# ForJadeForest/DistillCLIP

Hardware: AMD Instinct MI355X
Metric: image-text pairs/sec (distill step) (higher is better)
Workload: dtype bf16; 1 GPU; l_clip.yaml dual distill: ViT-B/32 CLIP teacher -> weight-shared ViT(6x768,24h,R2) + text(4x768,12h,R2) students, 224px/77tok, losses out_l1+out_cos+0.1*cos_diff, fwd+loss+bwd+AdamW; global_batch=512, batch_per_gpu=512, parallelism=dp1, gradient_exchange=none, negatives=local (reference training_step semantics), optimizer_in_step=True, teacher_residual=fp16, saved_gelu_derivative=u8 fixed point, clock_probe=True

## Files before the change

### distillclip_amd/csrc/attention_mix.hip

```cpp
#include <math.h>
#include <stdlib.h>
#include "common.h"

#define DEVFN __device__ __forceinline__
#define DEVMEM __device__ __forceinline__
typedef __attribute__((ext_vector_type(8))) _Float16 f16x8;

namespace hw {
DEVFN f32x4 mfma_bf16(bf16x8 a, bf16x8 b, f32x4 c) { return __builtin_amdgcn_mfma_f32_16x16x32_bf16(a, b, c, 0, 0, 0); }
DEVFN f32x4 mfma_f16(f16x8 a, f16x8 b, f32x4 c) { return __builtin_amdgcn_mfma_f32_16x16x32_f16(a, b, c, 0, 0, 0); }
DEVFN float exp2(float x) { return __builtin_amdgcn_exp2f(x); }
DEVFN float log2(float x) { return __builtin_amdgcn_logf(x); }
DEVFN bool any(bool p) { return __builtin_amdgcn_ballot_w64(p) != 0; }
DEVFN void lds_fence() { wave_lds_fence(); }
DEVFN void block_sync() { __syncthreads(); }
template <int OFF>
DEVFN bf16x8 lds_read_frag(const char* p) {
    bf16x8 v;
    asm volatile("ds_read_b128 %0, %1 offset:%2" : "=v"(v) : "v"((unsigned)(uintptr_t)p), "n"(OFF));
    return v;
}
template <int N, int GF>
DEVFN void lds_wait_frags(bf16x8 (&f)[GF]) {
    static_assert(GF == 4 || GF == 8, "fragment group of 4 or 8");
    if constexpr (GF == 8)
        asm volatile("s_waitcnt lgkmcnt(%8)" : "+v"(f[0]), "+v"(f[1]), "+v"(f[2]), "+v"(f[3]), "+v"(f[4]), "+v"(f[5]), "+v"(f[6]), "+v"(f[7]) : "n"(N));
    else
        asm volatile("s_waitcnt lgkmcnt(%4)" : "+v"(f[0]), "+v"(f[1]), "+v"(f[2]), "+v"(f[3]) : "n"(N));
}
DEVFN void pin_acc(bf16x8& v) { asm volatile("" : "+a"(v)); }
DEVFN unsigned long long clock() { return __builtin_readcyclecounter(); }
template <class T8> DEVFN void keep_alive(const T8 (&f)[4]) { mfma_keep_alive(f); }
template <class T8> DEVFN void keep_alive(const T8& f) { mfma_keep_alive(f); }
DEVFN void mfma_src_guard() { __builtin_amdgcn_sched_barrier(0); asm volatile("s_nop 7\n\ts_nop 3" ::: "memory"); __builtin_amdgcn_sched_barrier(0); }
DEVFN void sched_fence() { __builtin_amdgcn_sched_barrier(0); }
typedef __attribute__((address_space(3))) void lds_void;
typedef __attribute__((address_space(1))) const void gbl_void;
DEVFN void dma16(const void* src, char* dst) { __builtin_amdgcn_global_load_lds((gbl_void*)src, (lds_void*)dst, 16, 0, 0); }
template <int N> DEVFN void dma_wait() { asm volatile("s_waitcnt vmcnt(%0)" ::"n"(N) : "memory"); }
}

#include "attn_mix_wave.h"

namespace {

constexpr int BWD_MAX_WG = 256;

DEVFN int pick_tile(const int32_t* pick, int b, int N) {
    const int it = (pick[b] - b * N) >> 4;
    return __builtin_amdgcn_readfirstlane(min(max(it, 0), (N - 1) >> 4));
}

template <int H, int HD, int OCC, bool PICK = false>
__global__ __launch_bounds__(256, OCC) void attn_mix_fwd_kernel(amix::FwdArgs p, const int32_t* pick) {
    using C = amix::Cfg<H, HD>;
    extern __shared__ __attribute__((aligned(16))) char smem[];
    const int lane = threadIdx.x & 63;
    const int wave = __builtin_amdgcn_readfirstlane(threadIdx.x >> 6);
    const int item = blockIdx.x * 4 + wave;
    if (item >= (PICK ? p.B : p.B * p.QT)) return;
    const int b = PICK ? item : item / p.QT, it = PICK ? pick_tile(pick, b, p.N) : item - b * p.QT;
    const unsigned long long te = p.stamps ? hw::clock() : 0;
    char* lds = smem + wave * amix::fwd_lds_per_wave<C>();
    amix::zero_block_init<C>(lds, lane);
    amix::FwdWeights<C> w;
    amix::fwd_load_weights<C>(p, lane, w);
    if (p.stamps && lane == 0) {
        p.stamps[12 * (long)item + 8] = hw::clock() - te;
        p.stamps[12 * (long)item + 10] = __builtin_amdgcn_s_memrealtime();
    }
    amix::fwd_item<C>(p, b, it, lane, w, lds);
    if (p.stamps && lane == 0) p.stamps[12 * (long)item + 11] = __builtin_amdgcn_s_memrealtime();
}

template <class C, bool PASS_B>
DEVFN void bwd_wave_pick(const amix::BwdArgs& p, const int32_t* pick, int wg, int nwg, int wave, int nwave, int lane, char* lds_all) {
    using namespace amix;
    constexpr int RT = C::RT, HP = C::HP;
    constexpr int PER_WAVE = bwd_lds_per_wave<C>(), TILE_OFF = bwd_tile_off<C>();
    char* lds = lds_all + wave * PER_WAVE;
    for (int o = lane * 16; o < 2 * WG_TILE; o += 64 * 16) *(u32x4*)(lds + TILE_OFF + o) = u32x4{0u, 0u, 0u, 0u};
    zero_block_init<C>(lds, lane);
    BwdWeights<C> w;
    bwd_load_weights<C, PASS_B>(p, lane, w);
    f32x4 acc[RT][RT];
#pragma unroll
    for (int t = 0; t < RT; ++t)
#pragma unroll
        for (int u = 0; u < RT; ++u) acc[t][u] = f32x4{0.f, 0.f, 0.f, 0.f};
    for (int b = wg * nwave + wave; b < p.B; b += nwg * nwave) bwd_item<C, PASS_B>(p, b, pick_tile(pick, b, p.N), lane, w, acc, lds);
    hw::lds_fence();
    float* mine = (float*)(lds + TILE_OFF);
    const int c = lane & 15, g4 = lane >> 4;
#pragma unroll
    for (int t = 0; t < RT; ++t)
#pragma unroll
        for (int u = 0; u < RT; ++u)
#pragma unroll
            for (int r = 0; r < 4; ++r) mine[(16 * t + 4 * g4 + r) * HP + 16 * u + c] = acc[t][u][r];
    hw::block_sync();
    float* out = p.partial + ((long)wg * 2 + (PASS_B ? 0 : 1)) * HP * HP;
    for (int idx = wave * 64 + lane; idx < HP * HP; idx += nwave * 64) {
        float s = 0.f;
        for (int v = 0; v < nwave; ++v) s += ((const float*)(lds_all + v * PER_WAVE + TILE_OFF))[idx];
        out[idx] = s;
    }
}

template <int H, int HD, bool PASS_B, bool PICK = false>
__global__ __launch_bounds__(256) void attn_mix_bwd_kernel(amix::BwdArgs p, const int32_t* pick) {
    using C = amix::Cfg<H, HD>;
    extern __shared__ __attribute__((aligned(16))) char smem[];
    const int lane = threadIdx.x & 63;
    const int wave = __builtin_amdgcn_readfirstlane(threadIdx.x >> 6);
    if constexpr (PICK) bwd_wave_pick<C, PASS_B>(p, pick, blockIdx.x, gridDim.x, wave, 4, lane, smem);
    else amix::bwd_wave<C, PASS_B>(p, blockIdx.x, gridDim.x, wave, 4, lane, smem);
}

__global__ __launch_bounds__(256) void attn_mix_wgrad_reduce_kernel(const float* __restrict__ partial, int nwg, int H, int HP, float* dWl, float* dWw) {
    __shared__ float part[4];
    const int idx = blockIdx.x;
    const int which = idx / (H * H), gh = idx - which * H * H, g = gh / H, h = gh - g * H;
    const int w = threadIdx.x;
    float v = w < nwg ? partial[((size_t)w * 2 + which) * HP * HP + g * HP + h] : 0.f;
    v = wave_sum(v);
    if ((w & 63) == 0) part[w >> 6] = v;
    __syncthreads();
    if (w == 0) {
        float* dst = which == 0 ? dWl : dWw;
        dst[gh] += (part[0] + part[1]) + (part[2] + part[3]);
    }
}

unsigned long long* g_fwd_stamps = nullptr;
unsigned long long* g_bwd_stamps[2] = {nullptr, nullptr};

}

#define MIX_DISPATCH(Hv, HDv, ...)                                                     \
    switch ((Hv) * 100 + (HDv)) {                                                      \
        case 232: { constexpr int HH = 2, HD_ = 32; typedef amix::Cfg<HH, HD_> CC; __VA_ARGS__; break; }              \
        case 264: { constexpr int HH = 2, HD_ = 64; typedef amix::Cfg<HH, HD_> CC; __VA_ARGS__; break; }              \
        case 432: { constexpr int HH = 4, HD_ = 32; typedef amix::Cfg<HH, HD_> CC; __VA_ARGS__; break; }              \
        case 464: { constexpr int HH = 4, HD_ = 64; typedef amix::Cfg<HH, HD_> CC; __VA_ARGS__; break; }              \
        case 832: { constexpr int HH = 8, HD_ = 32; typedef amix::Cfg<HH, HD_> CC; __VA_ARGS__; break; }              \
        case 864: { constexpr int HH = 8, HD_ = 64; typedef amix::Cfg<HH, HD_> CC; __VA_ARGS__; break; }              \
        case 1232: { constexpr int HH = 12, HD_ = 32; typedef amix::Cfg<HH, HD_> CC; __VA_ARGS__; break; }            \
        case 1264: { constexpr int HH = 12, HD_ = 64; typedef amix::Cfg<HH, HD_> CC; __VA_ARGS__; break; }            \
        case 2432: { constexpr int HH = 24, HD_ = 32; typedef amix::Cfg<HH, HD_> CC; __VA_ARGS__; break; }            \
        default: dclip_set_error("attn_mix: no instantiation for H=%d hd=%d", (int)(Hv), (int)(HDv)); return DCLIP_EINVAL; \
    }

extern "C" int dclip_attn_mix_supported(int64_t H, int64_t N, int64_t hd) {
    const bool shape = ((H == 2 || H == 4 || H == 8 || H == 12) && (hd == 32 || hd == 64)) || (H == 24 && hd == 32);
    return shape && H * hd <= 1024 && (H * hd) % 128 == 0 && N >= 1 && N <= 128;
}

extern "C" void dclip_attn_mix_debug_stamps(void* fwd, void* bwd_a, void* bwd_b) {
    g_fwd_stamps = (unsigned long long*)fwd;
    g_bwd_stamps[0] = (unsigned long long*)bwd_a;
    g_bwd_stamps[1] = (unsigned long long*)bwd_b;
}

static size_t partial_bytes(int64_t H) {
    const size_t HP = (size_t)((H + 15) / 16) * 16;
    return (size_t)BWD_MAX_WG * 2 * HP * HP * sizeof(float);
}
extern "C" size_t dclip_attn_mix_bwd_workspace_bytes(int64_t B, int64_t H, int64_t N) {
    return partial_bytes(H) + (((size_t)B * H * N * sizeof(float) + 255) & ~(size_t)255);
}

namespace {

int launch_mix_fwd(const char* who, const void* qkv, int64_t ld, const float* Wl, const float* Ww, void* R, float* stats, int64_t B, int64_t H,
                   int64_t N, int64_t Np, int64_t hd, float scale, const int32_t* pick, void* stream) {
    DCLIP_REQUIRE(qkv && Wl && Ww && R && stats && B > 0, "%s: null / empty argument", who);
    DCLIP_REQUIRE(dclip_attn_mix_supported(H, N, hd), "%s: unsupported shape H=%ld N=%ld hd=%ld", who, (long)H, (long)N, (long)hd);
    DCLIP_REQUIRE(Np == ((N + 7) & ~(int64_t)7) && ld % 8 == 0 && ld >= 3 * H * hd && ((uintptr_t)qkv % 16) == 0 && ((uintptr_t)R % 16) == 0,
                  "%s: misaligned buffers (Np = round_up(N, 8), 16-byte aligned qkv rows and R)", who);
    const int QT = (int)((N + 15) / 16);
    amix::FwdArgs p{(const bf16_t*)qkv, (long)ld, Wl, Ww, (bf16_t*)R, stats, (int)B, (int)N, (int)Np, QT, scale, pick ? nullptr : g_fwd_stamps};
    const int64_t nitem = pick ? B : B * QT;
    const dim3 grid((unsigned)((nitem + 3) / 4));
    const double rows = pick ? 16.0 : (double)N, el = (double)B * H * rows * Np;
    TraceScope tr(DCLIP_TRACE_ATTN, 4.0 * B * H * rows * N * hd + 8.0 * el * H, 2.0 * el + 2.0 * B * (N + rows) * H * hd, stream, (int)(B * H), (int)N, (int)hd, 7);
    if (pick) {
        MIX_DISPATCH(H, hd, hipLaunchKernelGGL((attn_mix_fwd_kernel<HH, HD_, 2, true>), grid, dim3(256), (size_t)4 * amix::fwd_lds_per_wave<CC>(),
                                               (hipStream_t)stream, p, pick));
    } else {
        MIX_DISPATCH(H, hd, hipLaunchKernelGGL((attn_mix_fwd_kernel<HH, HD_, 2>), grid, dim3(256), (size_t)4 * amix::fwd_lds_per_wave<CC>(),
                                               (hipStream_t)stream, p, nullptr));
    }
    return dclip_check_launch(who);
}

int launch_mix_bwd(const char* who, const void* qkv, int64_t ld, const void* dO, int64_t ldo, const float* Wl, const float* Ww, const float* stats,
                   void* dS, float* dWl, float* dWw, void* workspace, size_t ws_bytes, int64_t B, int64_t H, int64_t N, int64_t Np, int64_t hd,
                   float scale, const int32_t* pick, void* stream) {
    DCLIP_REQUIRE(qkv && dO && Wl && Ww && stats && dS && dWl && dWw && workspace && B > 0, "%s: null / empty argument", who);
    DCLIP_REQUIRE(dclip_attn_mix_supported(H, N, hd), "%s: unsupported shape H=%ld N=%ld hd=%ld", who, (long)H, (long)N, (long)hd);
    DCLIP_REQUIRE(Np == ((N + 7) & ~(int64_t)7) && ld % 8 == 0 && ldo % 8 == 0 && ld >= 3 * H * hd && ldo >= H * hd && ((uintptr_t)qkv % 16) == 0 &&
                      ((uintptr_t)dO % 16) == 0 && ((uintptr_t)dS % 16) == 0 && ((uintptr_t)workspace % 16) == 0,
                  "%s: misaligned buffers", who);
    DCLIP_REQUIRE(ws_bytes >= dclip_attn_mix_bwd_workspace_bytes(B, H, N), "%s: workspace too small (%zu < %zu)", who, ws_bytes,
                  dclip_attn_mix_bwd_workspace_bytes(B, H, N));
    const int QT = (int)((N + 15) / 16);
    const int HP = (int)((H + 15) / 16) * 16;
    const int64_t nitem = pick ? B : B * QT;
    int blocks = (int)((nitem + 3) / 4);
    if (blocks > BWD_MAX_WG) blocks = BWD_MAX_WG;
    amix::BwdArgs p{(const bf16_t*)qkv, (long)ld, (const bf16_t*)dO, (long)ldo, Wl, Ww, stats, (bf16_t*)dS, (float*)workspace,
                    (float*)((char*)workspace + partial_bytes(H)), (int)B, (int)N, (int)Np, QT, scale, pick ? nullptr : g_bwd_stamps[0]};
    const double rows = pick ? 16.0 : (double)N, el = (double)B * H * rows * Np;
    TraceScope tr(DCLIP_TRACE_ATTN, 8.0 * B * H * rows * N * hd + 20.0 * el * H, 2.0 * el + 4.0 * B * (N + rows) * H * hd, stream, (int)(B * H), (int)N, (int)hd, 8);
    if (pick) {
        MIX_DISPATCH(H, hd, hipLaunchKernelGGL((attn_mix_bwd_kernel<HH, HD_, false, true>), dim3(blocks), dim3(256), (size_t)4 * amix::bwd_lds_per_wave<CC>(),
                                               (hipStream_t)stream, p, pick));
        MIX_DISPATCH(H, hd, hipLaunchKernelGGL((attn_mix_bwd_kernel<HH, HD_, true, true>), dim3(blocks), dim3(256), (size_t)4 * amix::bwd_lds_per_wave<CC>(),
                                               (hipStream_t)stream, p, pick));
    } else {
        MIX_DISPATCH(H, hd, hipLaunchKernelGGL((attn_mix_bwd_kernel<HH, HD_, false>), dim3(blocks), dim3(256), (size_t)4 * amix::bwd_lds_per_wave<CC>(),
                                               (hipStream_t)stream, p, nullptr));
        p.stamps = g_bwd_stamps[1];
        MIX_DISPATCH(H, hd, hipLaunchKernelGGL((attn_mix_bwd_kernel<HH, HD_, true>), dim3(blocks), dim3(256), (size_t)4 * amix::bwd_lds_per_wave<CC>(),
                                               (hipStream_t)stream, p, nullptr));
    }
    static_assert(BWD_MAX_WG <= 256, "one partial per thread of the reduction block");
    hipLaunchKernelGGL(attn_mix_wgrad_reduce_kernel, dim3((unsigned)(2 * H * H)), dim3(256), 0, (hipStream_t)stream,
                       (const float*)workspace, blocks, (int)H, HP, dWl, dWw);
    return dclip_check_launch(who);
}

}

extern "C" int dclip_attn_mix_fwd(const void* qkv, int64_t ld, const float* Wl, const float* Ww, void* R, float* stats, int64_t B,
                                  int64_t H, int64_t N, int64_t Np, int64_t hd, float scale, void* stream) {
    return launch_mix_fwd("dclip_attn_mix_fwd", qkv, ld, Wl, Ww, R, stats, B, H, N, Np, hd, scale, nullptr, stream);
}

extern "C" int dclip_attn_mix_bwd(const void* qkv, int64_t ld, const void* dO, int64_t ldo, const float* Wl, const float* Ww,
                                  const float* stats, void* dS, float* dWl, float* dWw, void* workspace, size_t ws_bytes, int64_t B,
                                  int64_t H, int64_t N, int64_t Np, int64_t hd, float scale, void* stream) {
    return launch_mix_bwd("dclip_attn_mix_bwd", qkv, ld, dO, ldo, Wl, Ww, stats, dS, dWl, dWw, workspace, ws_bytes, B, H, N, Np, hd, scale, nullptr, stream);
}

extern "C" int dclip_attn_mix_fwd_rows(const void* qkv, int64_t ld, const float* Wl, const float* Ww, void* R, float* stats, int64_t B,
                                       int64_t H, int64_t N, int64_t Np, int64_t hd, float scale, const int32_t* pick, void* stream) {
    DCLIP_REQUIRE(pick, "dclip_attn_mix_fwd_rows: null pick");
    return launch_mix_fwd("dclip_attn_mix_fwd_rows", qkv, ld, Wl, Ww, R, stats, B, H, N, Np, hd, scale, pick, stream);
}

extern "C" int dclip_attn_mix_bwd_rows(const void* qkv, int64_t ld, const void* dO, int64_t ldo, const float* Wl, const float* Ww,
                                       const float* stats, void* dS, float* dWl, float* dWw, void* workspace, size_t ws_bytes, int64_t B,
                                       int64_t H, int64_t N, int64_t Np, int64_t hd, float scale, const int32_t* pick, void* stream) {
    DCLIP_REQUIRE(pick, "dclip_attn_mix_bwd_rows: null pick");
    return launch_mix_bwd("dclip_attn_mix_bwd_rows", qkv, ld, dO, ldo, Wl, Ww, stats, dS, dWl, dWw, workspace, ws_bytes, B, H, N, Np, hd, scale, pick, stream);
}
```

### distillclip_amd/csrc/common.h

```cpp
#pragma once
#include <hip/hip_runtime.h>
#include <stdint.h>

typedef __bf16 bf16_t;
typedef __attribute__((ext_vector_type(8))) __bf16 bf16x8;
typedef __attribute__((ext_vector_type(4))) __bf16 bf16x4;
typedef __attribute__((ext_vector_type(2))) __bf16 bf16x2;
typedef __attribute__((ext_vector_type(8))) _Float16 f16x8;
typedef __attribute__((ext_vector_type(4))) _Float16 f16x4;
typedef __attribute__((ext_vector_type(4))) short s16x4;
typedef __attribute__((ext_vector_type(4))) float f32x4;
typedef __attribute__((ext_vector_type(16))) float f32x16;
typedef __attribute__((ext_vector_type(4))) unsigned int u32x4;

#include "dclip.h"

void dclip_set_error(const char* fmt, ...);

#define DCLIP_REQUIRE(cond, ...)                 \
    do {                                          \
        if (!(cond)) {                            \
            dclip_set_error(__VA_ARGS__);         \
            return DCLIP_EINVAL;                  \
        }                                         \
    } while (0)

extern "C" int dclip_rows_pick(const void* src, void* dst, const int32_t* idx, int64_t B, int64_t row_bytes, void* stream);
extern "C" int dclip_rows_expand(const void* src, void* dst, const int32_t* idx, int64_t B, int64_t N, int64_t row_bytes, void* stream);

extern "C" int dclip_cast_bf16_pad(const float* src, void* dst, int64_t R, int64_t C, int64_t ldd, void* stream);

bool dclip_trace_open(int kind, double flops, double bytes, void* stream, int* slot, int d0 = 0, int d1 = 0, int d2 = 0, int d3 = 0);
void dclip_trace_close(int slot, void* stream);
struct TraceScope {
    int slot = -1; void* st;
    TraceScope(int kind, double flops, double bytes, void* stream, int d0 = 0, int d1 = 0, int d2 = 0, int d3 = 0) : st(stream) {
        if (!dclip_trace_open(kind, flops, bytes, stream, &slot, d0, d1, d2, d3)) slot = -1;
    }
    ~TraceScope() { if (slot >= 0) dclip_trace_close(slot, st); }
};
#define DCLIP_TRACE_GEMM_NT 0
#define DCLIP_TRACE_GEMM_TN 1
#define DCLIP_TRACE_LAYERNORM 2
#define DCLIP_TRACE_LOSS 3
#define DCLIP_TRACE_ATTN 4
#define DCLIP_TRACE_LN_BWD 5

void dclip_explain_hip_error(const char* what, int hip_error, const char* hip_text);
static inline int dclip_check_launch(const char* what) {
    hipError_t e = hipGetLastError();
    if (e != hipSuccess) {
        dclip_explain_hip_error(what, (int)e, hipGetErrorString(e));
        return DCLIP_ELAUNCH;
    }
    return DCLIP_OK;
}

static inline int grid_for(int64_t work, int per_block = 256, int cap = 2048 * 4) {
    int64_t g = (work + per_block - 1) / per_block;
    return (int)(g < 1 ? 1 : (g > cap ? cap : g));
}

static inline size_t dclip_up256(size_t x) { return (x + 255) & ~(size_t)255; }
static inline bool dclip_aligned16(const void* p) { return ((uintptr_t)p % 16) == 0; }
struct Bump {
    char* base; size_t off;
    explicit Bump(void* b) : base((char*)b), off(0) {}
    template <class T> T* take(size_t n) {
        T* p = base ? (T*)(base + off) : nullptr;
        off += dclip_up256(n * sizeof(T));
        return p;
    }
};

__device__ __forceinline__ float bf2f(bf16_t x) { return (float)x; }
__device__ __forceinline__ bf16_t f2bf(float x) { return (bf16_t)x; }

__device__ __forceinline__ float wave_sum(float v) {
#pragma unroll
    for (int o = 32; o > 0; o >>= 1) v += __shfl_xor(v, o);
    return v;
}
__device__ __forceinline__ float wave_max(float v) {
#pragma unroll
    for (int o = 32; o > 0; o >>= 1) v = fmaxf(v, __shfl_xor(v, o));
    return v;
}

__device__ __forceinline__ void wave_lds_fence() { __builtin_amdgcn_wave_barrier(); asm volatile("" ::: "memory"); __builtin_amdgcn_wave_barrier(); }

template <class T> __device__ __forceinline__ void mfma_keep_alive(const T& f) { asm volatile("" :: "v"(f)); }
template <class T> __device__ __forceinline__ void mfma_keep_alive(const T (&f)[2]) { asm volatile("" :: "v"(f[0]), "v"(f[1])); }
template <class T> __device__ __forceinline__ void mfma_keep_alive(const T (&f)[4]) { asm volatile("" :: "v"(f[0]), "v"(f[1]), "v"(f[2]), "v"(f[3])); }

__device__ __forceinline__ float quick_gelu_f(float x) { return x * __builtin_amdgcn_rcpf(1.f + __expf(-1.702f * x)); }
__device__ __forceinline__ float erf_tail(float ax_over_sqrt2, float phi) {
    const float t = __builtin_amdgcn_rcpf(fmaf(0.3275911f, ax_over_sqrt2, 1.f));
    float p = fmaf(1.061405429f, t, -1.453152027f);
    p = fmaf(p, t, 1.421413741f);
    p = fmaf(p, t, -0.284496736f);
    p = fmaf(p, t, 0.254829592f);
    return p * t * phi;
}
__device__ __forceinline__ float gelu_erf_f(float x) {
    const float phi = __expf(-0.5f * x * x);
    const float tail = erf_tail(fabsf(x) * 0.70710678118654752f, phi);
    const float cdf = x >= 0.f ? 1.f - 0.5f * tail : 0.5f * tail;
    return x * cdf;
}
__device__ __forceinline__ float dgelu_erf_f(float x) {
    const float phi = __expf(-0.5f * x * x);
    const float tail = erf_tail(fabsf(x) * 0.70710678118654752f, phi);
    const float cdf = x >= 0.f ? 1.f - 0.5f * tail : 0.5f * tail;
    return fmaf(x * phi, 0.3989422804014327f, cdf);
}

__device__ __forceinline__ void gelu_erf_both_f(float x, float& g, float& dg) {
    const float phi = __expf(-0.5f * x * x);
    const float tail = erf_tail(fabsf(x) * 0.70710678118654752f, phi);
    const float cdf = x >= 0.f ? 1.f - 0.5f * tail : 0.5f * tail;
    g = x * cdf;
    dg = fmaf(x * phi, 0.3989422804014327f, cdf);
}

#define DCLIP_DG_LO (-0.13f)
#define DCLIP_DG_STEP (1.26f / 255.f)
__device__ __forceinline__ unsigned dg_pack4(float a, float b, float c, float d) {
    const float inv = 255.f / 1.26f, off = 0.13f * (255.f / 1.26f);
    unsigned r = 0;
    r = __builtin_amdgcn_cvt_pk_u8_f32(__builtin_rintf(fmaf(a, inv, off)), 0, r);
    r = __builtin_amdgcn_cvt_pk_u8_f32(__builtin_rintf(fmaf(b, inv, off)), 1, r);
    r = __builtin_amdgcn_cvt_pk_u8_f32(__builtin_rintf(fmaf(c, inv, off)), 2, r);
    r = __builtin_amdgcn_cvt_pk_u8_f32(__builtin_rintf(fmaf(d, inv, off)), 3, r);
    return r;
}
__device__ __forceinline__ float dg_unpack(unsigned w, int byte) {
    return fmaf((float)((w >> (8 * byte)) & 0xffu), DCLIP_DG_STEP, DCLIP_DG_LO);
}

__device__ __forceinline__ bf16x8 frag_halves(s16x4 lo, s16x4 hi) {
    union { struct { s16x4 lo, hi; } s; bf16x8 v; } u;
    u.s.lo = lo; u.s.hi = hi;
    return u.v;
}

typedef __attribute__((address_space(3))) s16x4 lds_s16x4;
template <int ROWB>
__device__ __forceinline__ bf16x8 tr_frag(const char* tile, int r0, int x0, int lane) {
    const int g = lane >> 4, q = (lane >> 2) & 3, pp = lane & 3;
    const char* a0 = tile + (r0 + 8 * g + q) * ROWB + (x0 + 4 * pp) * 2;
    return frag_halves(__builtin_amdgcn_ds_read_tr16_b64_v4i16((lds_s16x4*)a0), __builtin_amdgcn_ds_read_tr16_b64_v4i16((lds_s16x4*)(a0 + 4 * ROWB)));
}

__device__ __forceinline__ int xcd_remap(int bid, int nwg) {
    const int q = nwg >> 3, r = nwg & 7, x = bid & 7;
    return (x < r ? x * (q + 1) : r * (q + 1) + (x - r) * q) + (bid >> 3);
}
```

### distillclip_amd/csrc/encoder.cpp

```cpp
#include <math.h>
#include <stdlib.h>
#include <string.h>
#include <new>
#include <vector>
#include "common.h"

namespace {

#define CK(expr)                      \
    do {                              \
        int _rc = (expr);             \
        if (_rc != DCLIP_OK) return _rc; \
    } while (0)

enum { P_PER_TBLOCK = 12, P_PER_SBLOCK = 8, P_PER_SREPEAT = 6 };

struct Plan {
    dclip_encoder_cfg c;
    int D, H, hd, N, Np, F, E, L, R;
    int K;
    int Kp;
    bool student, image, compressed;
    bool mixing;
    bool train;
    struct EmbP { int table, w, bias, cls, pos, ln_w, ln_b; } emb;
    int p_blocks;
    struct HeadP { int norm_w, norm_b, head_w, head_b; } head;
    int n_params;
    struct BlockW { int64_t qkv, qkv_t, proj, proj_t, fc1, fc1_t, fc2, fc2_t; };
    std::vector<BlockW> bw;
    int64_t w_embed, w_embed_t, w_head, w_head_t, w_total;
};

int64_t wtake(int64_t& off, int64_t n) { int64_t o = off; off += (n + 127) & ~(int64_t)127; return o; }

bool make_plan(const dclip_encoder_cfg& c, Plan& p) {
    p.c = c;
    p.student = c.kind == 1; p.train = c.kind != 0; p.image = c.modality == 0; p.mixing = p.student && c.head_mix;
    p.D = c.width; p.H = c.heads; p.N = c.tokens; p.F = c.mlp_dim; p.E = c.out_dim; p.L = c.layers; p.R = c.repeats;
    if (c.kind < 0 || c.kind > 2 || c.modality < 0 || c.modality > 1) { dclip_set_error("encoder: bad kind/modality"); return false; }
    if (p.D <= 0 || p.H <= 0 || p.D % p.H) { dclip_set_error("encoder: width %d not divisible by heads %d", p.D, p.H); return false; }
    p.hd = p.D / p.H;
    if (p.hd != 32 && p.hd != 64) { dclip_set_error("encoder: head dim %d unsupported (32 or 64)", p.hd); return false; }
    if (p.D % 64 || p.F % 64 || p.E % 64 || p.D > 1024) { dclip_set_error("encoder: width/mlp/out dims must be multiples of 64, width <= 1024"); return false; }
    const bool long_ok = c.kind == 0 && p.image && !c.causal && p.hd == 64;
    if (p.N <= 0 || p.N > (long_ok ? 640 : 128)) {
        if (long_ok) dclip_set_error("encoder: tokens must be in 1..640 for a frozen image tower (got %d)", p.N);
        else if (p.N > 128 && c.kind != 0) dclip_set_error("encoder: tokens must be in 1..128 for a trainable tower (kind %d; got %d): only frozen image towers run longer sequences", c.kind, p.N);
        else if (p.N > 128 && !p.image) dclip_set_error("encoder: tokens must be in 1..128 for a text tower (got %d): only frozen image towers run longer sequences", p.N);
        else if (p.N > 128) dclip_set_error("encoder: tokens must be in 1..128 for a causal or head-dim-%d tower (got %d): longer sequences need a non-causal tower with head dim 64", p.hd, p.N);
        else dclip_set_error("encoder: tokens must be in 1..128 (got %d)", p.N);
        return false;
    }
    if (p.L <= 0 || p.R <= 0 || (!p.student && p.R != 1)) { dclip_set_error("encoder: bad layers/repeats"); return false; }
    p.Np = (p.N + 7) & ~7;
    p.compressed = !p.image && c.embed_rank > 0;
    p.K = p.Kp = 0;
    if (p.image) {
        if (c.patch <= 0 || c.resolution < c.patch || c.in_chans <= 0) { dclip_set_error("encoder: bad patch geometry"); return false; }
        const int g = c.resolution / c.patch;
        if (g * g + 1 != p.N) { dclip_set_error("encoder: tokens %d != (res/patch)^2 + 1 = %d", p.N, g * g + 1); return false; }
        p.K = c.in_chans * c.patch * c.patch;
        p.Kp = p.K;
        if (p.K % 64) {
            if (p.train) { dclip_set_error("encoder: in_chans*patch^2 = %d must be a multiple of 64 in a trainable tower", p.K); return false; }
            if (c.patch % 2) { dclip_set_error("encoder: patch %d must be even", c.patch); return false; }
            p.Kp = (p.K + 63) & ~63;
        }
    } else {
        if (c.vocab <= 0) { dclip_set_error("encoder: vocab required for text"); return false; }
        if (p.compressed && c.embed_rank % 64) { dclip_set_error("encoder: embed_rank must be a multiple of 64"); return false; }
        if (p.compressed && !p.student) { dclip_set_error("encoder: a compressed token embedding exists for the weight-shared student only (kind 1)"); return false; }
        if (p.compressed) p.K = p.Kp = c.embed_rank;
    }
    if (p.mixing && p.H != 2 && p.H != 4 && p.H != 8 && p.H != 12 && p.H != 24) {
        dclip_set_error("encoder: head count %d unsupported by the head-mixing kernels", p.H); return false;
    }
    int n = 0;
    Plan::EmbP& em = p.emb;
    em = Plan::EmbP{-1, -1, -1, -1, -1, -1, -1};
    if (p.image) {
        em.w = n++;
        if (p.student) em.bias = n++;
        em.cls = n++; em.pos = n++;
        if (!p.student) { em.ln_w = n++; em.ln_b = n++; }
    } else {
        em.table = n++;
        if (p.compressed) { em.w = n++; em.bias = n++; }
        em.pos = n++;
    }
    p.p_blocks = n;
    n += p.student ? p.L * (P_PER_SBLOCK + p.R * P_PER_SREPEAT) : p.L * P_PER_TBLOCK;
    p.head.norm_w = n++; p.head.norm_b = n++; p.head.head_w = n++;
    p.head.head_b = p.student ? n++ : -1;
    p.n_params = n;
    int64_t off = 0;
    const int64_t D = p.D, F = p.F, E = p.E;
    p.bw.resize(p.L);
    for (int l = 0; l < p.L; ++l) {
        auto& b = p.bw[l];
        b.qkv = wtake(off, 3 * D * D); b.proj = wtake(off, D * D); b.fc1 = wtake(off, F * D); b.fc2 = wtake(off, D * F);
        if (p.train) { b.qkv_t = wtake(off, 3 * D * D); b.proj_t = wtake(off, D * D); b.fc1_t = wtake(off, F * D); b.fc2_t = wtake(off, D * F); }
        else b.qkv_t = b.proj_t = b.fc1_t = b.fc2_t = -1;
    }
    p.w_embed = p.w_embed_t = -1;
    if (em.w >= 0) p.w_embed = wtake(off, D * p.Kp);
    if (p.compressed) p.w_embed_t = wtake(off, D * p.K);
    p.w_head = wtake(off, E * D);
    p.w_head_t = p.train ? wtake(off, E * D) : -1;
    p.w_total = off;
    return true;
}

enum class AttnPath { Fused, Mix, Unfused };
inline AttnPath attn_path(const Plan& p, bool training) {
    static const int mode = [] { const char* e = getenv("DCLIP_ATTN_MIX"); return e ? atoi(e) : 1; }();
    if (!training && !p.mixing) return AttnPath::Fused;
    if (p.mixing && mode != 0 && !p.c.causal && dclip_attn_mix_supported(p.H, p.N, p.hd) != 0) return AttnPath::Mix;
    return AttnPath::Unfused;
}

struct ExecSave {
    void* x_mid;
    float* mean1; float* rstd1; float* mean2; float* rstd2;
    bf16_t *h1, *qkv, *ctx, *h2, *u;
    uint8_t* z;
    float* S;
    bf16_t* P;
    bf16_t* Rm;
    float* stats;
};

void take_scores(Bump& b, const Plan& p, AttnPath path, int64_t B, int64_t N, int64_t Np, ExecSave& s) {
    const int64_t SN = B * p.H * N * Np;
    const bool unfused = path == AttnPath::Unfused;
    s.S = unfused ? b.take<float>(SN) : nullptr;
    s.P = unfused ? b.take<bf16_t>(SN) : nullptr;
    s.Rm = p.mixing ? b.take<bf16_t>(SN) : s.P;
    s.stats = path == AttnPath::Mix ? b.take<float>(B * p.H * N) : nullptr;
}

struct RowSet {
    bf16_t* ctx;
    void *xin, *x_mid, *xout;
    bf16_t *h2, *u;
    float *mean2, *rstd2; uint8_t* z;
    int64_t rows;
};

struct Work {
    std::vector<void*> X;
    bool h16;
    std::vector<ExecSave> ex;
    bf16_t* patches;
    float* tok_table;
    int32_t* pick;
    float *meanf, *rstdf;
    bf16_t* hf;
    void* x0;
    float *mean0, *rstd0;
    float* G0;
    float* G; bf16_t* Gb;
    bf16_t *gb_f2, *gb_pr;
    bf16_t *dbig, *dh, *dqkv, *dout;
    bf16_t* dR;
    bf16_t* dS;
    float* tok_sum; float* demb;
    float* wg_dummy;
    float* mix_ws; size_t mix_ws_bytes;
    void* tn_ws; size_t tn_ws_bytes;
    RowSet compact;
    bf16_t* ctx_full;
    float* Gc;
    AttnPath path;
    size_t bytes;
};

void layout(const Plan& p, int64_t B, bool training, void* base, Work& w, int64_t N = 0) {
    Bump b(base);
    w = Work{};
    if (N <= 0) N = p.N;
    const int64_t Npad = (N + 7) & ~(int64_t)7;
    const int64_t M = B * N, D = p.D, F = p.F, SN = B * p.H * N * Npad;
    const int nex = p.L * p.R;
    const bool save = p.train && training;
    w.path = attn_path(p, save);
    const bool mix = w.path == AttnPath::Mix, unfused = w.path == AttnPath::Unfused;
    w.X.assign(nex + 1, nullptr);
    w.ex.assign(nex, ExecSave{});
    ExecSave shared{};
    void* xs = nullptr;
    w.h16 = !p.train;
    if (!save) {
        xs = w.h16 ? (void*)b.take<_Float16>(M * D) : (void*)b.take<float>(M * D);
        shared.x_mid = xs;
        shared.h1 = b.take<bf16_t>(M * D); shared.qkv = b.take<bf16_t>(M * 3 * D);
        take_scores(b, p, w.path, B, N, Npad, shared);
        shared.ctx = b.take<bf16_t>(M * D); shared.h2 = shared.h1; shared.u = b.take<bf16_t>(M * F);
    }
    for (int e = 0; e <= nex; ++e) w.X[e] = save ? (void*)b.take<float>(M * D) : xs;
    for (int e = 0; e < nex; ++e) {
        if (!save) { w.ex[e] = shared; continue; }
        ExecSave& s = w.ex[e];
        s.x_mid = b.take<float>(M * D);
        s.mean1 = b.take<float>(M); s.rstd1 = b.take<float>(M); s.mean2 = b.take<float>(M); s.rstd2 = b.take<float>(M);
        s.qkv = b.take<bf16_t>(M * 3 * D);
        take_scores(b, p, w.path, B, N, Npad, s);
        s.z = b.take<uint8_t>(M * F);
        if (e % p.R == 0) {
            bf16_t* h1 = b.take<bf16_t>(p.R * M * D); bf16_t* ctx = b.take<bf16_t>(p.R * M * D);
            bf16_t* h2 = b.take<bf16_t>(p.R * M * D); bf16_t* u = b.take<bf16_t>(p.R * M * F);
            for (int r = 0; r < p.R; ++r) {
                ExecSave& t = w.ex[e + r];
                t.h1 = h1 + r * M * D; t.ctx = ctx + r * M * D; t.h2 = h2 + r * M * D; t.u = u + r * M * F;
            }
        }
    }
    {
        const ExecSave& s = w.ex[nex - 1];
        if (save) {
            w.ctx_full = s.h2;
            w.compact = RowSet{s.ctx, w.X[nex], s.x_mid, w.X[nex], s.h2, s.u, s.mean2, s.rstd2, s.z, B};
        } else {
            w.ctx_full = shared.ctx;
            bf16_t* cctx = b.take<bf16_t>(B * D);
            const size_t es = w.h16 ? 2 : 4;
            void* xr = b.take<char>(B * D * es); void* xmc = b.take<char>(B * D * es); void* xoc = b.take<char>(B * D * es);
            w.compact = RowSet{cctx, xr, xmc, xoc, shared.h1, shared.u, nullptr, nullptr, nullptr, B};
        }
        w.Gc = save ? b.take<float>(B * D) : nullptr;
    }
    w.patches = p.emb.w >= 0 ? b.take<bf16_t>(M * p.Kp) : nullptr;
    w.tok_table = b.take<float>((int64_t)N * D);
    w.pick = b.take<int32_t>(B);
    w.meanf = b.take<float>(B); w.rstdf = b.take<float>(B);
    w.hf = b.take<bf16_t>(B * D);
    const bool pre_ln = p.emb.ln_w >= 0, pre = save && pre_ln;
    w.x0 = pre_ln ? (w.h16 ? (void*)b.take<_Float16>(M * D) : (void*)b.take<float>(M * D)) : nullptr;
    w.mean0 = pre ? b.take<float>(M) : nullptr; w.rstd0 = pre ? b.take<float>(M) : nullptr; w.G0 = pre ? b.take<float>(M * D) : nullptr;
    if (save) {
        w.G = b.take<float>(M * D); w.Gb = b.take<bf16_t>(M * D);
        w.gb_f2 = b.take<bf16_t>(p.R * M * D); w.gb_pr = b.take<bf16_t>(p.R * M * D);
        w.dbig = b.take<bf16_t>(p.R * M * F); w.dh = b.take<bf16_t>(M * D); w.dqkv = b.take<bf16_t>(p.R * M * 3 * D);
        w.dR = unfused ? b.take<bf16_t>(SN) : nullptr; w.dS = b.take<bf16_t>(SN); w.dout = b.take<bf16_t>(B * p.E);
        w.tok_sum = b.take<float>((int64_t)N * D);
        w.wg_dummy = mix ? b.take<float>(2 * p.H * p.H) : nullptr;
        w.mix_ws_bytes = mix ? dclip_attn_mix_bwd_workspace_bytes(B, p.H, N) : 0;
        w.mix_ws = w.mix_ws_bytes ? (float*)b.take<char>(w.mix_ws_bytes) : nullptr;
        w.tn_ws_bytes = dclip_gemm_tn_workspace_bytes();
        w.tn_ws = b.take<char>(w.tn_ws_bytes);
        w.demb = p.compressed ? b.take<float>(M * p.K) : nullptr;
    }
    w.bytes = b.off;
}

inline RowSet full_rows(const Work& w, int ei, int64_t M) {
    const ExecSave& s = w.ex[ei];
    return RowSet{s.ctx, w.X[ei], s.x_mid, w.X[ei + 1], s.h2, s.u, s.mean2, s.rstd2, s.z, M};
}

inline const float* PF(const void* const* params, int i) { return i < 0 ? nullptr : (const float*)params[i]; }

inline int wsplits(int64_t M, int64_t P, int64_t Q) {
    const double tiles = (double)((P + 127) / 128) * (double)((Q + 127) / 128);
    const int smax = (int)((M + 255) / 256);
    int best = 1;
    double best_t = 1e30;
    for (int s = 1; s <= smax && s <= 64; ++s) {
        const double blocks = tiles * s;
        const double rounds = ceil(blocks / 512.0);
        const double t_mm = rounds * (2.0 * 128 * 128 * ((double)M / s)) / 1.76e12;
        const double t_at = 0.5 * s * (double)P * Q * 4.0 / 1.3e12;
        const double t = t_mm + t_at + 2e-6;
        if (t < best_t) { best_t = t; best = s; }
    }
    return best;
}

inline int gemm(const void* A, int64_t lda, const void* Bw, int64_t ldb, void* C, int64_t ldc, int64_t M, int64_t N, int64_t K,
                const float* bias, int act, const void* aux_in, void* aux_out, const void* res, int64_t ldr, int out_dtype,
                int64_t row_group, const float* rowadd, void* st) {
    return dclip_gemm_nt(A, lda, Bw, ldb, C, ldc, M, N, K, 1.f, bias, act, aux_in, aux_out, res, ldr, out_dtype, row_group, rowadd, nullptr, st);
}

inline int ln_stream(bool h16, const void* x, int64_t ldx, const int32_t* ridx, const float* g, const float* b, void* y, int64_t ldy, int out_dtype,
                     float* mean, float* rstd, int64_t M, int64_t D, void* st) {
    if (h16) return dclip_layernorm_fwd_f16(x, ldx, ridx, g, b, y, ldy, out_dtype, mean, rstd, M, D, 1e-5f, st);
    return dclip_layernorm_fwd((const float*)x, ldx, ridx, g, b, y, ldy, out_dtype, mean, rstd, M, D, 1e-5f, st);
}

inline int export_stream(bool h16, const void* src, float* dst, int64_t n, void* st) {
    if (h16) return dclip_cast_f16_f32(src, dst, n, st);
    if (hipMemcpyAsync(dst, src, (size_t)n * 4, hipMemcpyDeviceToDevice, (hipStream_t)st) != hipSuccess) {
        dclip_set_error("dclip_encoder_forward: hidden-state export failed");
        return DCLIP_ELAUNCH;
    }
    return DCLIP_OK;
}

int attn_forward(AttnPath path, const Plan& p, const ExecSave& s, const float* wl, const float* ww, int64_t B, int64_t N, const int32_t* pick,
                 void* st) {
    const int64_t D = p.D, H = p.H, hd = p.hd, Np = (N + 7) & ~(int64_t)7;
    const float scale = 1.f / sqrtf((float)hd);
    if (path == AttnPath::Fused) {
        if (N <= 128 && pick) return dclip_attn_fused_fwd_rows(s.qkv, 3 * D, s.ctx, D, B, H, N, hd, scale, p.c.causal, pick, st);
        if (N <= 128) return dclip_attn_fused_fwd(s.qkv, 3 * D, s.ctx, D, B, H, N, hd, scale, p.c.causal, st);
        return dclip_attn_stream_fwd(s.qkv, 3 * D, s.ctx, D, B, H, N, hd, scale, st);
    }
    const int blk = path == AttnPath::Mix ? 1 : 0;
    if (path == AttnPath::Mix) {
        if (pick) CK(dclip_attn_mix_fwd_rows(s.qkv, 3 * D, wl, ww, s.Rm, s.stats, B, H, N, Np, hd, scale, pick, st));
        else CK(dclip_attn_mix_fwd(s.qkv, 3 * D, wl, ww, s.Rm, s.stats, B, H, N, Np, hd, scale, st));
    } else {
        CK(dclip_attn_nt(s.qkv, 3 * D, s.qkv + D, 3 * D, s.S, 1, B, H, N, Np, hd, scale, st));
        CK(dclip_attn_softmax_fwd(s.S, wl, ww, wl ? s.P : nullptr, s.Rm, B, H, N, Np, p.c.causal, st));
    }
    if (pick) return dclip_attn_nn_rows(s.Rm, s.qkv + 2 * D, 3 * D, s.ctx, D, B, H, N, Np, hd, 1.f, blk, pick, 0, st);
    return dclip_attn_nn(s.Rm, s.qkv + 2 * D, 3 * D, s.ctx, D, B, H, N, Np, hd, 1.f, blk, st);
}

struct MapGrad { const float* d_score; const float* d_prob; void* scratch; size_t scratch_bytes; };
int attn_backward(AttnPath path, const Plan& p, const ExecSave& s, const Work& w, const float* wl, const float* ww, float* gl, float* gw,
                  const bf16_t* dctx, bf16_t* dqkv, int64_t B, const MapGrad* mg, const int32_t* pick, void* st) {
    const int64_t D = p.D, H = p.H, hd = p.hd, N = p.N, Np = p.Np;
    const float scale = 1.f / sqrtf((float)hd);
    const int blk = path == AttnPath::Mix ? 1 : 0;
    if (pick) {
        CK(dclip_attn_tn_rows(s.Rm, dctx, D, dqkv + 2 * D, 3 * D, B, H, N, Np, hd, 1.f, blk, pick, st));
        if (path == AttnPath::Mix) {
            CK(dclip_attn_mix_bwd_rows(s.qkv, 3 * D, dctx, D, wl, ww, s.stats, w.dS, gl ? gl : w.wg_dummy, gw ? gw : w.wg_dummy + H * H,
                                       w.mix_ws, w.mix_ws_bytes, B, H, N, Np, hd, scale, pick, st));
        } else {
            CK(dclip_attn_nt(dctx, D, s.qkv + 2 * D, 3 * D, w.dR, 0, B, H, N, Np, hd, 1.f, st));
            CK(dclip_attn_softmax_bwd(w.dR, s.P, s.S, 0, wl, ww, w.dS, gl, gw, B, H, N, Np, st));
        }
        CK(dclip_attn_nn_rows(w.dS, s.qkv + D, 3 * D, dqkv, 3 * D, B, H, N, Np, hd, scale, blk, pick, 1, st));
        return dclip_attn_tn_rows(w.dS, s.qkv, 3 * D, dqkv + D, 3 * D, B, H, N, Np, hd, scale, blk, pick, st);
    }
    CK(dclip_attn_tn(s.Rm, dctx, D, dqkv + 2 * D, 3 * D, B, H, N, Np, hd, 1.f, blk, st));
    if (path == AttnPath::Mix) {
        CK(dclip_attn_mix_bwd(s.qkv, 3 * D, dctx, D, wl, ww, s.stats, w.dS, gl ? gl : w.wg_dummy, gw ? gw : w.wg_dummy + H * H,
                              w.mix_ws, w.mix_ws_bytes, B, H, N, Np, hd, scale, st));
    } else {
        CK(dclip_attn_nt(dctx, D, s.qkv + 2 * D, 3 * D, w.dR, 0, B, H, N, Np, hd, 1.f, st));
        CK(dclip_attn_softmax_bwd(w.dR, s.P, s.S, 0, wl, ww, w.dS, gl, gw, B, H, N, Np, st));
    }
    if (mg) CK(dclip_attn_maps_bwd(s.qkv, 3 * D, wl, mg->d_score, mg->d_prob, w.dS, blk, gl, mg->scratch, mg->scratch_bytes, B, H, N, Np, hd,
                                   scale, p.c.causal, st));
    CK(dclip_attn_nn(w.dS, s.qkv + D, 3 * D, dqkv, 3 * D, B, H, N, Np, hd, scale, blk, st));
    return dclip_attn_tn(w.dS, s.qkv, 3 * D, dqkv + D, 3 * D, B, H, N, Np, hd, scale, blk, st);
}

}

enum : uint32_t { RUN_SEEDS_CLEAR = 1u, RUN_PRUNED = 2u, RUN_PRUNED_ATTN = 4u };

struct dclip_encoder { Plan p; };

extern "C" dclip_encoder* dclip_encoder_create(const dclip_encoder_cfg* cfg) {
    if (!cfg) { dclip_set_error("dclip_encoder_create: null cfg"); return nullptr; }
    dclip_encoder* e = new (std::nothrow) dclip_encoder();
    if (!e) { dclip_set_error("dclip_encoder_create: out of host memory"); return nullptr; }
    if (!make_plan(*cfg, e->p)) { delete e; return nullptr; }
    return e;
}

extern "C" void dclip_encoder_destroy(dclip_encoder* e) { delete e; }
extern "C" int64_t dclip_encoder_num_params(const dclip_encoder* e) { return e ? e->p.n_params : -1; }
extern "C" size_t dclip_encoder_wcache_bytes(const dclip_encoder* e) { return e ? dclip_up256((size_t)e->p.w_total * 2) : 0; }

extern "C" size_t dclip_encoder_workspace_bytes(const dclip_encoder* e, int64_t B, int training) {
    if (!e || B <= 0) return 0;
    Work w;
    layout(e->p, B, training != 0, nullptr, w);
    return w.bytes;
}

namespace {
struct BX { int n1w, n1b, n2w, n2b, qkvw, qkvb, prw, prb, f1w, f1b, f2w, f2b, cl, cw; };
inline BX bexec(const Plan& p, int l, int r) {
    if (!p.student) {
        const int b = p.p_blocks + l * P_PER_TBLOCK;
        return BX{b, b + 1, b + 6, b + 7, b + 2, b + 3, b + 4, b + 5, b + 8, b + 9, b + 10, b + 11, -1, -1};
    }
    const int b = p.p_blocks + l * (P_PER_SBLOCK + p.R * P_PER_SREPEAT), q = b + P_PER_SBLOCK + r * P_PER_SREPEAT;
    return BX{q, q + 1, q + 2, q + 3, b, b + 1, b + 2, b + 3, b + 4, b + 5, b + 6, b + 7, q + 4, q + 5};
}

struct EP { const float *n1w, *n1b, *n2w, *n2b, *bq, *bp, *b1, *b2, *wl, *ww; };
inline EP exec_params(const Plan& p, const void* const* params, int l, int r) {
    const BX bx = bexec(p, l, r);
    EP e{PF(params, bx.n1w), PF(params, bx.n1b), PF(params, bx.n2w), PF(params, bx.n2b), PF(params, bx.qkvb), PF(params, bx.prb),
         PF(params, bx.f1b), PF(params, bx.f2b), nullptr, nullptr};
    if (p.mixing) { e.wl = PF(params, bx.cl); e.ww = PF(params, bx.cw); }
    return e;
}

int exec_attn(const Plan& p, AttnPath path, const ExecSave& s, const bf16_t* W, int l, const EP& e, bool h16, const void* xin, int64_t B,
              int64_t N, const int32_t* pick, void* st) {
    const int64_t D = p.D, M = B * N;
    CK(ln_stream(h16, xin, D, nullptr, e.n1w, e.n1b, s.h1, D, DCLIP_OUT_BF16, s.mean1, s.rstd1, M, D, st));
    CK(gemm(s.h1, D, W + p.bw[l].qkv, D, s.qkv, 3 * D, M, 3 * D, D, e.bq, 0, nullptr, nullptr, nullptr, 0, DCLIP_OUT_BF16, 0, nullptr, st));
    return attn_forward(path, p, s, e.wl, e.ww, B, N, pick, st);
}

int exec_mlp(const Plan& p, const bf16_t* W, int l, const EP& e, bool h16, const RowSet& rs, void* st) {
    const int64_t D = p.D, F = p.F, rows = rs.rows;
    const auto& bw = p.bw[l];
    const int sdt = h16 ? DCLIP_OUT_F16 : DCLIP_OUT_F32;
    const int act = p.student ? (rs.z ? DCLIP_ACT_GELU_SAVE : DCLIP_ACT_GELU) : (rs.z ? DCLIP_ACT_QUICKGELU_SAVE : DCLIP_ACT_QUICKGELU);
    CK(gemm(rs.ctx, D, W + bw.proj, D, rs.x_mid, D, rows, D, D, e.bp, 0, nullptr, nullptr, rs.xin, D, sdt, 0, nullptr, st));
    CK(ln_stream(h16, rs.x_mid, D, nullptr, e.n2w, e.n2b, rs.h2, D, DCLIP_OUT_BF16, rs.mean2, rs.rstd2, rows, D, st));
    CK(gemm(rs.h2, D, W + bw.fc1, D, rs.u, F, rows, F, D, e.b1, act, nullptr, rs.z, nullptr, 0, DCLIP_OUT_BF16, 0, nullptr, st));
    return gemm(rs.u, F, W + bw.fc2, F, rs.xout, D, rows, D, F, e.b2, 0, nullptr, nullptr, rs.x_mid, D, sdt, 0, nullptr, st);
}

size_t llo_scratch(const Plan& p, AttnPath path, bool h16, int64_t B, void* base, void* xin, ExecSave& t, RowSet& rs) {
    Bump b(base);
    const int64_t N = p.N, M = B * N, D = p.D, F = p.F;
    const size_t es = h16 ? 2 : 4;
    t = ExecSave{};
    t.h1 = b.take<bf16_t>(M * D); t.h2 = t.h1;
    t.qkv = b.take<bf16_t>(M * 3 * D);
    take_scores(b, p, path, B, N, p.Np, t);
    t.ctx = b.take<bf16_t>(M * D);
    t.x_mid = b.take<char>(M * D * es);
    t.u = b.take<bf16_t>(M * F);
    rs = RowSet{t.ctx, xin, t.x_mid, b.take<char>(M * D * es), t.h2, t.u, nullptr, nullptr, nullptr, M};
    return b.off;
}

inline bool prune_last_enabled() {
    static const int v = [] { const char* e = getenv("DCLIP_PRUNE_LAST"); return e ? atoi(e) : 1; }();
    return v != 0;
}
inline bool prune_attn_enabled() {
    static const int v = [] { const char* e = getenv("DCLIP_PRUNE_ATTN"); return e ? atoi(e) : 1; }();
    return v != 0;
}

template <class T> struct ExecMaps { std::vector<T*> score, prob; uint64_t score_bits = 0, prob_bits = 0; };
template <class T>
int exec_maps(const Plan& p, const dclip_attn_maps* maps, T* const* score, T* const* prob, const dclip_encoder_run* rec, const char* fn,
              ExecMaps<T>& out) {
    const int nex = p.L * p.R;
    out.score.assign(nex, nullptr); out.prob.assign(nex, nullptr);
    if (!maps || !maps->n) return DCLIP_OK;
    DCLIP_REQUIRE(maps->n > 0 && maps->exec, "%s: maps need n > 0 execution indices", fn);
    for (int k = 0; k < maps->n; ++k) {
        const int ei = maps->exec[k];
        DCLIP_REQUIRE(ei >= 0 && ei < nex, "%s: map %d: block execution %d out of range 0..%d", fn, k, ei, nex - 1);
        T* sm = score ? score[k] : nullptr;
        T* pm = prob ? prob[k] : nullptr;
        if (!rec) {
            DCLIP_REQUIRE(ei < 64, "%s: map %d: block execution %d: maps are exported for executions 0..63 only", fn, k, ei);
        } else {
            const bool had_s = ei < 64 && (rec->score_maps >> ei & 1), had_p = ei < 64 && (rec->prob_maps >> ei & 1);
            DCLIP_REQUIRE((!sm || had_s) && (!pm || had_p), "%s: a gradient for the %s map of block execution %d, which the forward did not export",
                          fn, sm && !had_s ? "score" : "probability", ei);
        }
        if (sm) { out.score[ei] = sm; out.score_bits |= (uint64_t)1 << ei; }
        if (pm) { out.prob[ei] = pm; out.prob_bits |= (uint64_t)1 << ei; }
    }
    return DCLIP_OK;
}
}

extern "C" int dclip_encoder_prepare(const dclip_encoder* e, const void* const* params, void* wcache, void* st) {
    DCLIP_REQUIRE(e && params && wcache, "dclip_encoder_prepare: null argument");
    const Plan& p = e->p;
    bf16_t* W = (bf16_t*)wcache;
    const int64_t D = p.D, F = p.F, E = p.E;
    auto at = [&](int64_t off) -> void* { return off < 0 ? nullptr : (void*)(W + off); };
    std::vector<const float*> src; std::vector<void*> wb, wt; std::vector<int64_t> rr, cc;
    auto job = [&](const float* w, void* b, void* t, int64_t R, int64_t C) { src.push_back(w); wb.push_back(b); wt.push_back(t); rr.push_back(R); cc.push_back(C); };
    for (int l = 0; l < p.L; ++l) {
        const auto& b = p.bw[l];
        const BX bx = bexec(p, l, 0);
        job(PF(params, bx.qkvw), at(b.qkv), at(b.qkv_t), 3 * D, D);
        job(PF(params, bx.prw), at(b.proj), at(b.proj_t), D, D);
        job(PF(params, bx.f1w), at(b.fc1), at(b.fc1_t), F, D);
        job(PF(params, bx.f2w), at(b.fc2), at(b.fc2_t), D, F);
    }
    const bool pad_embed = p.Kp != p.K;
    if (p.emb.w >= 0 && !pad_embed) job(PF(params, p.emb.w), at(p.w_embed), at(p.w_embed_t), D, p.K);
    if (p.student) job(PF(params, p.head.head_w), at(p.w_head), at(p.w_head_t), E, D);
    else job(PF(params, p.head.head_w), at(p.w_head_t), at(p.w_head), D, E);
    for (size_t i = 0; i < src.size(); ++i) DCLIP_REQUIRE(src[i], "dclip_encoder_prepare: parameter %zu missing", i);
    if (pad_embed) {
        DCLIP_REQUIRE(PF(params, p.emb.w), "dclip_encoder_prepare: the patch-embedding weight is missing");
        CK(dclip_cast_bf16_pad(PF(params, p.emb.w), at(p.w_embed), D, p.K, p.Kp, st));
    }
    return dclip_cast_transpose_bf16_multi(src.data(), wb.data(), wt.data(), rr.data(), cc.data(), (int64_t)src.size(), st);
}

static int clear_backward_seeds(const Plan& p, const Work& w, int64_t M, int64_t B, bool pruned, void* st) {
    const int64_t D = p.D;
    hipStream_t hs = (hipStream_t)st;
    bf16_t* gb_last = w.gb_f2 + (int64_t)(p.R - 1) * M * D;
    const bool ok = pruned ? hipMemsetAsync(w.Gc, 0, (size_t)B * D * 4, hs) == hipSuccess
                           : hipMemsetAsync(w.G, 0, (size_t)M * D * 4, hs) == hipSuccess && hipMemsetAsync(gb_last, 0, (size_t)M * D * 2, hs) == hipSuccess;
    if (!ok) { dclip_set_error("dclip_encoder: clearing the backward seeds failed"); return DCLIP_ELAUNCH; }
    return DCLIP_OK;
}

extern "C" int dclip_encoder_forward(const dclip_encoder* e, const void* input, const void* patches, int64_t B, const void* const* params,
                                     const void* wcache, void* workspace, size_t ws_bytes, dclip_encoder_run* run, int training,
                                     float* last_representation, float* const* rep_out, float* emb_out, int64_t tokens_eff,
                                     const dclip_attn_maps* maps, void* st) {
    DCLIP_REQUIRE(e && (input || patches) && params && wcache && workspace && run && last_representation, "dclip_encoder_forward: null argument");
    DCLIP_REQUIRE(B > 0, "dclip_encoder_forward: empty batch");
    const Plan& p = e->p;
    const bf16_t* ext_patches = (const bf16_t*)patches;
    DCLIP_REQUIRE(!ext_patches || (p.image && ((uintptr_t)ext_patches % 16) == 0), "dclip_encoder_forward: patches: image towers only, 16-byte aligned rows");
    DCLIP_REQUIRE(!ext_patches || tokens_eff == 0, "dclip_encoder_forward: patches cannot be combined with tokens_eff");
    DCLIP_REQUIRE(!ext_patches || p.Kp == p.K, "dclip_encoder_forward: this tower pads its patch rows (%d -> %d columns) and cuts them itself: pass the images", p.K, p.Kp);
    DCLIP_REQUIRE(!training || p.train, "dclip_encoder_forward: the frozen teacher tower (kind 0) is inference-only");
    DCLIP_REQUIRE(tokens_eff == 0 || (!p.train && !p.image && p.c.causal && tokens_eff > 0 && tokens_eff <= p.N && !rep_out && !emb_out),
                  "dclip_encoder_forward: tokens_eff is only valid for the causal text teacher without hidden-state export");
    DCLIP_REQUIRE(!(maps && maps->n > 0 && maps->exec) || tokens_eff == 0,
                  "dclip_encoder_forward: attention maps cannot be exported from a caption prefix (tokens_eff)");
    DCLIP_REQUIRE(!(maps && maps->n > 0) || p.N <= 128,
                  "dclip_encoder_forward: attention maps cannot be exported from a tower of %d tokens (dclip_attn_maps_fwd / _bwd take N <= 128)", p.N);
    ExecMaps<float> xm;
    CK(exec_maps<float>(p, maps, maps ? maps->score : nullptr, maps ? maps->prob : nullptr, nullptr, "dclip_encoder_forward", xm));
    Work w;
    layout(p, B, training != 0, workspace, w, tokens_eff);
    DCLIP_REQUIRE(ws_bytes >= w.bytes, "dclip_encoder_forward: workspace too small (%zu < %zu)", ws_bytes, w.bytes);
    DCLIP_REQUIRE(((uintptr_t)workspace % 256) == 0 && ((uintptr_t)wcache % 256) == 0, "dclip_encoder_forward: buffers must be 256-byte aligned");
    const bf16_t* W = (const bf16_t*)wcache;
    const int64_t N = tokens_eff ? tokens_eff : p.N, D = p.D, F = p.F, E = p.E, M = B * N;
    const int nex = p.L * p.R;

    const Plan::EmbP& em = p.emb;
    const bool pre_ln = em.ln_w >= 0;
    const int sdt = w.h16 ? DCLIP_OUT_F16 : DCLIP_OUT_F32;
    if (em.w >= 0) {
        const bf16_t* rows = ext_patches ? ext_patches : w.patches;
        if (!p.image) CK(dclip_embed_gather((const int64_t*)input, p.N, PF(params, em.table), nullptr, w.patches, 0, M, N, p.K, st));
        else if (!ext_patches && p.Kp != p.K) CK(dclip_im2row_ld((const float*)input, w.patches, p.Kp, B, p.c.in_chans, p.c.resolution, p.c.patch, 1, st));
        else if (!ext_patches) CK(dclip_im2row((const float*)input, w.patches, B, p.c.in_chans, p.c.resolution, p.c.patch, 1, st));
        CK(dclip_token_table(PF(params, em.pos), PF(params, em.cls), PF(params, em.bias), w.tok_table, N, D, st));
        CK(gemm(rows, p.Kp, W + p.w_embed, p.Kp, pre_ln ? w.x0 : w.X[0], D, M, D, p.Kp, nullptr, 0, nullptr, nullptr, nullptr, 0, sdt, N, w.tok_table, st));
        if (pre_ln) CK(ln_stream(w.h16, w.x0, D, nullptr, PF(params, em.ln_w), PF(params, em.ln_b), w.X[0], D, sdt, w.mean0, w.rstd0, M, D, st));
    } else {
        CK(dclip_embed_gather((const int64_t*)input, p.N, PF(params, em.table), PF(params, em.pos), w.X[0], sdt, M, N, D, st));
    }

    if (emb_out) CK(export_stream(w.h16, pre_ln ? w.x0 : w.X[0], emb_out, M * D, st));

    CK(dclip_pick_index(p.image ? nullptr : (const int64_t*)input, p.N, w.pick, B, N, st));
    const bool prune = prune_last_enabled() && !(rep_out && rep_out[nex - 1]) && !xm.score[nex - 1] && !xm.prob[nex - 1];
    const bool prune_attn = prune && prune_attn_enabled() && N <= 128;
    for (int ei = 0; ei < nex; ++ei) {
        const int l = ei / p.R, r = ei % p.R;
        const ExecSave& s = w.ex[ei];
        const EP ep = exec_params(p, params, l, r);
        const bool compact = prune && ei == nex - 1;
        ExecSave sa = s;
        if (compact) sa.ctx = w.ctx_full;
        CK(exec_attn(p, w.path, sa, W, l, ep, w.h16, w.X[ei], B, N, compact && prune_attn ? w.pick : nullptr, st));
        if (xm.score[ei] || xm.prob[ei]) CK(dclip_attn_maps_fwd(s.qkv, 3 * D, ep.wl, xm.score[ei], xm.prob[ei], B, p.H, N, p.hd, 1.f / sqrtf((float)p.hd), p.c.causal, st));
        if (compact) {
            CK(dclip_rows_pick(w.ctx_full, w.compact.ctx, w.pick, B, D * 2, st));
            CK(dclip_rows_pick(w.X[ei], w.compact.xin, w.pick, B, D * (w.h16 ? 2 : 4), st));
        }
        CK(exec_mlp(p, W, l, ep, w.h16, compact ? w.compact : full_rows(w, ei, M), st));
        if (rep_out && rep_out[ei]) CK(export_stream(w.h16, w.X[ei + 1], rep_out[ei], M * D, st));
    }

    CK(ln_stream(w.h16, prune ? w.compact.xout : w.X[nex], D, prune ? nullptr : w.pick, PF(params, p.head.norm_w), PF(params, p.head.norm_b), w.hf, D,
                 DCLIP_OUT_BF16, w.meanf, w.rstdf, B, D, st));
    CK(gemm(w.hf, D, W + p.w_head, D, last_representation, E, B, E, D, PF(params, p.head.head_b), 0, nullptr, nullptr, nullptr, 0, DCLIP_OUT_F32, 0, nullptr, st));
    *run = dclip_encoder_run{(prune ? RUN_PRUNED : 0u) | (prune_attn ? RUN_PRUNED_ATTN : 0u), 0, 0, 0};
    if (training) {
        CK(clear_backward_seeds(p, w, M, B, prune, st));
        run->flags |= RUN_SEEDS_CLEAR;
        run->score_maps = xm.score_bits;
        run->prob_maps = xm.prob_bits;
    }
    return DCLIP_OK;
}

extern "C" size_t dclip_encoder_last_layer_output_scratch_bytes(const dclip_encoder* e, int64_t B, int training) {
    if (!e || B <= 0) return 0;
    const Plan& p = e->p;
    ExecSave t;
    RowSet rs;
    return llo_scratch(p, attn_path(p, p.train && training != 0), !p.train, B, nullptr, nullptr, t, rs);
}

extern "C" int dclip_encoder_last_layer_output(const dclip_encoder* e, int64_t B, const void* const* params, const void* wcache,
                                               void* workspace, size_t ws_bytes, const dclip_encoder_run* run, int training, void* scratch,
                                               float* out, void* st) {
    DCLIP_REQUIRE(e && params && wcache && workspace && run && scratch && out, "dclip_encoder_last_layer_output: null argument");
    DCLIP_REQUIRE(B > 0, "dclip_encoder_last_layer_output: empty batch");
    const Plan& p = e->p;
    DCLIP_REQUIRE(!training || p.train, "dclip_encoder_last_layer_output: the frozen teacher tower (kind 0) is inference-only");
    Work w;
    layout(p, B, training != 0, workspace, w);
    DCLIP_REQUIRE(ws_bytes >= w.bytes, "dclip_encoder_last_layer_output: workspace too small (%zu < %zu)", ws_bytes, w.bytes);
    const bf16_t* W = (const bf16_t*)wcache;
    const int64_t M = B * p.N, D = p.D, E = p.E;
    const int nex = p.L * p.R;
    const void* xlast = w.X[nex];
    if (run->flags & RUN_PRUNED) {
        ExecSave t;
        RowSet rs;
        const int ei = nex - 1, l = ei / p.R;
        llo_scratch(p, w.path, w.h16, B, scratch, w.X[ei], t, rs);
        const EP ep = exec_params(p, params, l, ei % p.R);
        CK(exec_attn(p, w.path, t, W, l, ep, w.h16, w.X[ei], B, p.N, nullptr, st));
        CK(exec_mlp(p, W, l, ep, w.h16, rs, st));
        xlast = rs.xout;
    }
    CK(ln_stream(w.h16, xlast, D, nullptr, PF(params, p.head.norm_w), PF(params, p.head.norm_b), scratch, D, DCLIP_OUT_BF16, nullptr, nullptr, M, D, st));
    CK(gemm(scratch, D, W + p.w_head, D, out, E, M, E, D, PF(params, p.head.head_b), 0, nullptr, nullptr, nullptr, 0, DCLIP_OUT_F32, 0, nullptr, st));
    return DCLIP_OK;
}

extern "C" int dclip_encoder_backward(const dclip_encoder* e, const void* input, const void* patches, int64_t B, const void* const* params,
                                      void* const* grads, const void* wcache, void* workspace, size_t ws_bytes, dclip_encoder_run* run,
                                      const float* d_last_representation, const float* const* d_rep, const float* d_emb,
                                      const dclip_attn_maps* maps, dclip_bucket_cb on_bucket, void* cb_user, void* st) {
    DCLIP_REQUIRE(e && (input || patches) && params && grads && wcache && workspace && run && d_last_representation, "dclip_encoder_backward: null argument");
    const Plan& p = e->p;
    const bf16_t* ext_patches = (const bf16_t*)patches;
    DCLIP_REQUIRE(!ext_patches || p.image, "dclip_encoder_backward: patches: image towers only");
    DCLIP_REQUIRE(p.train, "dclip_encoder_backward: the frozen teacher tower (kind 0) has no backward");
    ExecMaps<const float> gm;
    CK(exec_maps<const float>(p, maps, maps ? maps->d_score : nullptr, maps ? maps->d_prob : nullptr, run, "dclip_encoder_backward", gm));
    if (p.mixing && gm.prob_bits) {
        const size_t need = dclip_attn_maps_bwd_workspace_bytes(B, p.H, p.N);
        DCLIP_REQUIRE(maps->scratch && maps->scratch_bytes >= need,
                      "dclip_encoder_backward: probability-map gradients of a head-mixing tower need %zu bytes of maps scratch", need);
    }
    Work w;
    layout(p, B, true, workspace, w);
    DCLIP_REQUIRE(ws_bytes >= w.bytes, "dclip_encoder_backward: workspace too small");
    const bf16_t* W = (const bf16_t*)wcache;
    const int64_t N = p.N, D = p.D, F = p.F, E = p.E, M = B * N;
    const int nex = p.L * p.R;
    const bool pruned = (run->flags & RUN_PRUNED) != 0;
    DCLIP_REQUIRE(!pruned || !(d_rep && d_rep[nex - 1]),
                  "dclip_encoder_backward: a gradient for the hidden state of block execution %d, which the forward ran on the class / EOT "
                  "rows only (request that hidden state in the forward, or set DCLIP_PRUNE_LAST=0)", nex - 1);
    DCLIP_REQUIRE(!pruned || !(gm.score[nex - 1] || gm.prob[nex - 1]),
                  "dclip_encoder_backward: a map gradient for block execution %d, which the forward ran on the class / EOT rows only", nex - 1);
    auto GR = [&](int i) -> float* { return i < 0 ? nullptr : (float*)grads[i]; };
    hipStream_t hs = (hipStream_t)st;

    if (run->flags & RUN_SEEDS_CLEAR) run->flags &= ~RUN_SEEDS_CLEAR;
    else CK(clear_backward_seeds(p, w, M, B, pruned, st));
    CK(dclip_cast_bf16(d_last_representation, w.dout, B * E, st));
    if (p.student) {
        if (GR(p.head.head_w)) CK(dclip_gemm_tn_acc(w.dout, E, w.hf, D, GR(p.head.head_w), D, B, E, D, 1, w.tn_ws, w.tn_ws_bytes, st));
        if (GR(p.head.head_b)) CK(dclip_colsum_acc(w.dout, E, GR(p.head.head_b), B, E, st));
    } else if (GR(p.head.head_w)) {
        CK(dclip_gemm_tn_acc(w.hf, D, w.dout, E, GR(p.head.head_w), E, B, D, E, 1, w.tn_ws, w.tn_ws_bytes, st));
    }
    CK(gemm(w.dout, E, W + p.w_head_t, E, w.dh, D, B, D, E, nullptr, 0, nullptr, nullptr, nullptr, 0, DCLIP_OUT_BF16, 0, nullptr, st));
    const int R = p.R;
    bf16_t* gb_last = w.gb_f2 + (int64_t)(R - 1) * M * D;
    CK(dclip_layernorm_bwd(w.dh, D, 0, (const float*)(pruned ? w.compact.xout : w.X[nex]), D, pruned ? nullptr : w.pick, PF(params, p.head.norm_w), w.meanf,
                           w.rstdf, pruned ? w.Gc : w.G, D, gb_last, D, GR(p.head.norm_w), GR(p.head.norm_b), GR(bexec(p, (nex - 1) / p.R, 0).f2b), B, D, st));
    if (on_bucket) on_bucket(cb_user, 0);

    for (int ei = nex - 1; ei >= 0; --ei) {
        const int l = ei / p.R, r = ei % p.R;
        const auto& bw = p.bw[l];
        const ExecSave& s = w.ex[ei];
        const BX bx = bexec(p, l, r);
        const float *wl = nullptr, *ww = nullptr;
        float *gl = nullptr, *gw = nullptr;
        if (p.mixing) { wl = PF(params, bx.cl); ww = PF(params, bx.cw); gl = GR(bx.cl); gw = GR(bx.cw); }
        bf16_t* gb_f2 = w.gb_f2 + (int64_t)r * M * D;
        bf16_t* gb_pr = w.gb_pr + (int64_t)r * M * D;
        bf16_t* dbig = w.dbig + (int64_t)r * M * F;
        bf16_t* dqkv = w.dqkv + (int64_t)r * M * 3 * D;
        const int64_t MR = (int64_t)R * M;
        const ExecSave& s0 = w.ex[ei - r];
        const bool compact = pruned && ei == nex - 1;
        const RowSet rs = compact ? w.compact : full_rows(w, ei, M);
        const int64_t Mx = rs.rows;
        const int64_t MRw = pruned && l == p.L - 1 ? (int64_t)(R - 1) * M + B : MR;
        if (d_rep && d_rep[ei]) CK(dclip_axpy_f32(w.G, d_rep[ei], gb_f2, M * D, GR(bx.f2b), D, st));
        CK(dclip_gemm_nt(gb_f2, D, W + bw.fc2_t, D, dbig, F, Mx, F, D, 1.f, nullptr, DCLIP_ACT_MULAUX, rs.z, nullptr, nullptr, 0, DCLIP_OUT_BF16, 0, nullptr,
                         GR(bx.f1b), st));
        if (r == 0 && GR(bx.f2w)) CK(dclip_gemm_tn_acc(w.gb_f2, D, s0.u, F, GR(bx.f2w), F, MRw, D, F, wsplits(MRw, D, F), w.tn_ws, w.tn_ws_bytes, st));
        if (r == 0 && GR(bx.f1w)) CK(dclip_gemm_tn_acc(w.dbig, F, s0.h2, D, GR(bx.f1w), D, MRw, F, D, wsplits(MRw, F, D), w.tn_ws, w.tn_ws_bytes, st));
        CK(gemm(dbig, F, W + bw.fc1_t, F, w.dh, D, Mx, D, F, nullptr, 0, nullptr, nullptr, nullptr, 0, DCLIP_OUT_BF16, 0, nullptr, st));
        CK(dclip_layernorm_bwd(w.dh, D, 0, (const float*)rs.x_mid, D, nullptr, PF(params, bx.n2w), rs.mean2, rs.rstd2, compact ? w.Gc : w.G, D, gb_pr, D,
                               GR(bx.n2w), GR(bx.n2b), GR(bx.prb), Mx, D, st));
        if (r == 0 && GR(bx.prw)) CK(dclip_gemm_tn_acc(w.gb_pr, D, s0.ctx, D, GR(bx.prw), D, MRw, D, D, wsplits(MRw, D, D), w.tn_ws, w.tn_ws_bytes, st));
        bf16_t* dctx = w.dh;
        if (!compact) {
            CK(gemm(gb_pr, D, W + bw.proj_t, D, dctx, D, M, D, D, nullptr, 0, nullptr, nullptr, nullptr, 0, DCLIP_OUT_BF16, 0, nullptr, st));
        } else {
            bf16_t* dctx_c = dqkv;
            CK(gemm(gb_pr, D, W + bw.proj_t, D, dctx_c, D, B, D, D, nullptr, 0, nullptr, nullptr, nullptr, 0, DCLIP_OUT_BF16, 0, nullptr, st));
            CK(dclip_rows_expand(dctx_c, dctx, w.pick, B, N, D * 2, st));
            CK(dclip_rows_expand(w.Gc, w.G, w.pick, B, N, D * 4, st));
        }
        const MapGrad mg{gm.score[ei], gm.prob[ei], maps ? maps->scratch : nullptr, maps ? maps->scratch_bytes : 0};
        CK(attn_backward(w.path, p, s, w, wl, ww, gl, gw, dctx, dqkv, B, mg.d_score || mg.d_prob ? &mg : nullptr,
                         compact && (run->flags & RUN_PRUNED_ATTN) ? w.pick : nullptr, st));
        if (r == 0 && GR(bx.qkvw)) CK(dclip_gemm_tn_acc(w.dqkv, 3 * D, s0.h1, D, GR(bx.qkvw), D, MR, 3 * D, D, wsplits(MR, 3 * D, D), w.tn_ws, w.tn_ws_bytes, st));
        if (r == 0 && params[bx.qkvb] && GR(bx.qkvb)) CK(dclip_colsum_acc(w.dqkv, 3 * D, GR(bx.qkvb), MR, 3 * D, st));
        CK(gemm(dqkv, 3 * D, W + bw.qkv_t, 3 * D, w.dh, D, M, D, 3 * D, nullptr, 0, nullptr, nullptr, nullptr, 0, DCLIP_OUT_BF16, 0, nullptr, st));
        bf16_t* gb_next = ei > 0 ? w.gb_f2 + (int64_t)((ei - 1) % R) * M * D : w.Gb;
        CK(dclip_layernorm_bwd(w.dh, D, 0, (const float*)w.X[ei], D, nullptr, PF(params, bx.n1w), s.mean1, s.rstd1, w.G, D, gb_next, D, GR(bx.n1w), GR(bx.n1b),
                               ei > 0 ? GR(bexec(p, (ei - 1) / p.R, 0).f2b) : nullptr, M, D, st));
        if (r == 0 && on_bucket) on_bucket(cb_user, 1 + (p.L - 1 - l));
    }

    const Plan::EmbP& em = p.emb;
    const bool pre_ln = em.ln_w >= 0;
    if (d_emb && !pre_ln) CK(dclip_axpy_f32(w.G, d_emb, w.Gb, M * D, nullptr, D, st));
    if (hipMemsetAsync(w.tok_sum, 0, (size_t)N * D * 4, hs) != hipSuccess) { dclip_set_error("dclip_encoder_backward: memset failed"); return DCLIP_ELAUNCH; }
    const float* Ge = w.G;
    if (pre_ln) {
        if (hipMemsetAsync(w.G0, 0, (size_t)M * D * 4, hs) != hipSuccess) { dclip_set_error("dclip_encoder_backward: memset failed"); return DCLIP_ELAUNCH; }
        CK(dclip_layernorm_bwd(w.G, D, 1, (const float*)w.x0, D, nullptr, PF(params, em.ln_w), w.mean0, w.rstd0, w.G0, D, w.Gb, D, GR(em.ln_w), GR(em.ln_b),
                               nullptr, M, D, st));
        if (d_emb) CK(dclip_axpy_f32(w.G0, d_emb, w.Gb, M * D, nullptr, D, st));
        Ge = w.G0;
    }
    if (em.w >= 0) {
        const int64_t K = p.K;
        const bf16_t* rows = ext_patches ? ext_patches : w.patches;
        if (GR(em.w)) CK(dclip_gemm_tn_acc(w.Gb, D, rows, K, GR(em.w), K, M, D, K, wsplits(M, D, K), w.tn_ws, w.tn_ws_bytes, st));
        if (GR(em.bias) || GR(em.cls) || GR(em.pos)) {
            CK(dclip_batch_sum_acc(Ge, w.tok_sum, B, N, D, st));
            CK(dclip_token_table_bwd(w.tok_sum, GR(em.pos), GR(em.cls), GR(em.bias), N, D, p.image ? 1 : 0, st));
        }
        if (GR(em.table)) {
            CK(gemm(w.Gb, D, W + p.w_embed_t, D, w.demb, K, M, K, D, nullptr, 0, nullptr, nullptr, nullptr, 0, DCLIP_OUT_F32, 0, nullptr, st));
            CK(dclip_embed_scatter_add((const int64_t*)input, w.demb, 1, GR(em.table), M, K, p.c.vocab, st));
        }
    } else {
        if (GR(em.table)) CK(dclip_embed_scatter_add((const int64_t*)input, w.G, 1, GR(em.table), M, D, p.c.vocab, st));
        if (GR(em.pos)) {
            CK(dclip_batch_sum_acc(w.G, w.tok_sum, B, N, D, st));
            CK(dclip_token_table_bwd(w.tok_sum, GR(em.pos), nullptr, nullptr, N, D, 0, st));
        }
    }
    if (on_bucket) on_bucket(cb_user, p.L + 1);
    return DCLIP_OK;
}

extern "C" int32_t dclip_encoder_num_grad_buckets(const dclip_encoder* e) { return e ? e->p.L + 2 : -1; }
extern "C" int dclip_encoder_grad_bucket(const dclip_encoder* e, int32_t bucket, int32_t* first_param, int32_t* end_param) {
    DCLIP_REQUIRE(e && first_param && end_param, "dclip_encoder_grad_bucket: null argument");
    const Plan& p = e->p;
    DCLIP_REQUIRE(bucket >= 0 && bucket <= p.L + 1, "dclip_encoder_grad_bucket: bucket %d out of range 0..%d", bucket, p.L + 1);
    const int per_block = p.student ? P_PER_SBLOCK + p.R * P_PER_SREPEAT : P_PER_TBLOCK;
    if (bucket == 0) { *first_param = p.head.norm_w; *end_param = p.n_params; }
    else if (bucket == p.L + 1) { *first_param = 0; *end_param = p.p_blocks; }
    else { const int l = p.L - bucket; *first_param = p.p_blocks + l * per_block; *end_param = *first_param + per_block; }
    return DCLIP_OK;
}
```

### distillclip_amd/ops.py

```python
import torch

from ._lib import lib

ACT = {'none': 0, None: 0, 'quickgelu': 1, 'gelu': 2, 'dgelu': 3, 'mulaux': 4, 'gelu_save': 5, 'quickgelu_save': 6}
OUT_DTYPE = {torch.bfloat16: 0, torch.float32: 1, torch.float16: 2}
DG_LO, DG_STEP = -0.13, 1.26 / 255.0


def _p(t):
    return 0 if t is None else t.data_ptr()


def _stream():
    return torch.cuda.current_stream().cuda_stream


def _chk(*ts):
    for t in ts:
        if t is not None and not t.is_cuda:
            raise RuntimeError('distillclip_amd ops need CUDA(HIP) tensors; there is no CPU fallback')


def gemm_nt(a, b, *, bias=None, act=None, aux_in=None, aux_out=None, residual=None, out=None, out_dtype=torch.bfloat16,
            alpha=1.0, row_group=0, rowadd=None, out_rows=None, colsum=None):
    _chk(a, b, bias, aux_in, aux_out, residual, out, rowadd)
    assert a.dtype == torch.bfloat16 and b.dtype == torch.bfloat16 and a.dim() == 2 and b.dim() == 2
    assert a.stride(1) == 1 and b.stride(1) == 1
    M, K = a.shape
    N = b.shape[0]
    if out is None:
        rows = out_rows if out_rows is not None else M
        out = torch.empty((rows, N), dtype=out_dtype, device=a.device)
    assert out.stride(1) == 1
    ldr = residual.stride(0) if residual is not None else 0
    if act in ('gelu_save', 'quickgelu_save') and aux_out is not None:
        assert aux_out.dtype == torch.uint8 and aux_out.stride(0) == out.stride(0)
    if act == 'mulaux':
        assert aux_in.dtype == torch.uint8 and aux_in.stride(0) == out.stride(0)
    if residual is not None:
        assert residual.dtype == (torch.float16 if out.dtype == torch.float16 else torch.float32)
    lib().dclip_gemm_nt(_p(a), a.stride(0), _p(b), b.stride(0), _p(out), out.stride(0), M, N, K, float(alpha),
                        _p(bias), ACT[act], _p(aux_in), _p(aux_out), _p(residual), ldr,
                        OUT_DTYPE[out.dtype], row_group, _p(rowadd), _p(colsum), _stream())
    return out


_TN_WS = {}


def _tn_workspace(device):
    key = (device, _stream())
    ws = _TN_WS.get(key)
    if ws is None:
        ws = _TN_WS[key] = torch.empty(lib().dclip_gemm_tn_workspace_bytes(), dtype=torch.uint8, device=device)
    return ws


def gemm_tn_acc(a, b, dw, splits=4, workspace=True):
    _chk(a, b, dw)
    assert a.dtype == torch.bfloat16 and b.dtype == torch.bfloat16 and dw.dtype == torch.float32
    M, P = a.shape
    Q = b.shape[1]
    assert b.shape[0] == M and tuple(dw.shape) == (P, Q) and dw.stride(1) == 1
    ws = _tn_workspace(a.device) if workspace else None
    lib().dclip_gemm_tn_acc(_p(a), a.stride(0), _p(b), b.stride(0), _p(dw), dw.stride(0), M, P, Q, splits, _p(ws),
                            0 if ws is None else ws.numel(), _stream())
    return dw


def colsum_acc(x, db):
    _chk(x, db)
    assert x.dtype == torch.bfloat16 and db.dtype == torch.float32
    lib().dclip_colsum_acc(_p(x), x.stride(0), _p(db), x.shape[0], x.shape[1], _stream())
    return db


def layernorm_fwd(x, gamma, beta, *, row_index=None, out_dtype=torch.bfloat16, eps=1e-5, save_stats=True):
    _chk(x, gamma, beta, row_index)
    assert x.dtype in (torch.float32, torch.float16) and x.dim() == 2 and x.stride(1) == 1
    M = row_index.numel() if row_index is not None else x.shape[0]
    D = x.shape[1]
    y = torch.empty((M, D), dtype=out_dtype, device=x.device)
    mean = torch.empty(M, dtype=torch.float32, device=x.device) if save_stats else None
    rstd = torch.empty(M, dtype=torch.float32, device=x.device) if save_stats else None
    fn = lib().dclip_layernorm_fwd_f16 if x.dtype == torch.float16 else lib().dclip_layernorm_fwd
    fn(_p(x), x.stride(0), _p(row_index), _p(gamma), _p(beta), _p(y), D, OUT_DTYPE[out_dtype], _p(mean), _p(rstd), M, D, eps, _stream())
    return y, mean, rstd


def layernorm_bwd(dy, x, gamma, mean, rstd, dx_acc, *, row_index=None, dx_bf16=None, dgamma=None, dbeta=None, colsum=None):
    _chk(dy, x, gamma, mean, rstd, dx_acc, dx_bf16, dgamma, dbeta)
    M, D = dy.shape
    lib().dclip_layernorm_bwd(_p(dy), dy.stride(0), 1 if dy.dtype == torch.float32 else 0, _p(x), x.stride(0),
                              _p(row_index), _p(gamma), _p(mean), _p(rstd), _p(dx_acc), dx_acc.stride(0), _p(dx_bf16),
                              dx_bf16.stride(0) if dx_bf16 is not None else 0, _p(dgamma), _p(dbeta), _p(colsum), M, D, _stream())


def attn_nt(a, lda, bm, ldb, B, H, N, hd, alpha=1.0, out_dtype=torch.float32):
    Np = (N + 7) // 8 * 8
    c = torch.empty((B, H, N, Np), dtype=out_dtype, device=a.device)
    lib().dclip_attn_nt(_p(a), lda, _p(bm), ldb, _p(c), 1 if out_dtype == torch.float32 else 0, B, H, N, Np, hd, alpha,
                        _stream())
    return c


def _score_dims(a):
    if a.dim() == 5:
        B, H, nq, N, four = a.shape
        assert four == 4
        return B, H, N, nq * 4, 1
    B, H, N, Np = a.shape
    return B, H, N, Np, 0


def attn_nn(a, bm, ldb, c, ldc, hd, alpha=1.0):
    B, H, N, Np, blocked = _score_dims(a)
    lib().dclip_attn_nn(_p(a), _p(bm), ldb, _p(c), ldc, B, H, N, Np, hd, alpha, blocked, _stream())


def attn_tn(a, bm, ldb, c, ldc, hd, alpha=1.0):
    B, H, N, Np, blocked = _score_dims(a)
    lib().dclip_attn_tn(_p(a), _p(bm), ldb, _p(c), ldc, B, H, N, Np, hd, alpha, blocked, _stream())


def attn_nn_rows(a, bm, ldb, c, ldc, hd, pick, alpha=1.0, fill_zero=False):
    _chk(pick)
    B, H, N, Np, blocked = _score_dims(a)
    lib().dclip_attn_nn_rows(_p(a), _p(bm), ldb, _p(c), ldc, B, H, N, Np, hd, alpha, blocked, _p(pick), 1 if fill_zero else 0, _stream())


def attn_tn_rows(a, bm, ldb, c, ldc, hd, pick, alpha=1.0):
    _chk(pick)
    B, H, N, Np, blocked = _score_dims(a)
    lib().dclip_attn_tn_rows(_p(a), _p(bm), ldb, _p(c), ldc, B, H, N, Np, hd, alpha, blocked, _p(pick), _stream())


def unblock_scores(a):
    B, H, nq, N, _ = a.shape
    return a.permute(0, 1, 3, 2, 4).reshape(B, H, N, nq * 4)


def attn_softmax_fwd(s, wl=None, ww=None, causal=False, save_p=False):
    B, H, N, Np = s.shape
    r = torch.empty((B, H, N, Np), dtype=torch.bfloat16, device=s.device)
    p = torch.empty_like(r) if save_p else None
    lib().dclip_attn_softmax_fwd(_p(s), _p(wl), _p(ww), _p(p), _p(r), B, H, N, Np, 1 if causal else 0, _stream())
    return p, r


def attn_softmax_bwd(dr, p, s, wl=None, ww=None, dwl=None, dww=None):
    B, H, N, Np = dr.shape
    ds = torch.empty_like(dr)
    lib().dclip_attn_softmax_bwd(_p(dr), _p(p), _p(s), 1 if (s is not None and s.dtype == torch.bfloat16) else 0, _p(wl), _p(ww), _p(ds),
                                 _p(dwl), _p(dww), B, H, N, Np, _stream())
    return ds


LOSS_SLOTS = {'out_l1': 0, 'out_cos': 1, 'out_kl': 2, 'out_ce': 3, 'cos_diff': 4, 'hard_label': 5, 'soft_label': 6,
              'logits_mse': 7}


def distill_loss(s_img, t_img, s_txt=None, t_txt=None, *, weights, temperature=None, row0=None, rows=None, gathered_stats=None,
                 stats_only=False):
    import ctypes
    _chk(s_img, t_img, s_txt, t_txt)
    B, E = s_img.shape
    two = s_txt is not None
    cfg = [0.0] * 10
    for k, w in weights.items():
        cfg[LOSS_SLOTS[k]] = float(w)
    cfg[8] = float(temperature or 0.0)
    cfg[9] = 1.0 if two else 0.0
    cfg_arr = (ctypes.c_float * 10)(*cfg)
    ws_bytes = lib().dclip_distill_loss_workspace(B, E)
    ws = torch.empty(ws_bytes, dtype=torch.uint8, device=s_img.device)
    out = torch.empty(16, dtype=torch.float32, device=s_img.device)
    nrow = B if rows is None else int(rows)
    d_i = torch.empty((nrow, E), dtype=torch.float32, device=s_img.device)
    d_t = torch.empty((nrow, E), dtype=torch.float32, device=s_img.device) if two else None
    if rows is None:
        lib().dclip_distill_loss(_p(s_img), _p(t_img), _p(s_txt), _p(t_txt), B, E, ctypes.cast(cfg_arr, ctypes.c_void_p),
                                 _p(out), _p(d_i), _p(d_t), _p(ws), ws_bytes, _stream())
    else:
        stats = torch.empty((6, nrow), dtype=torch.float32, device=s_img.device) if stats_only else None
        if gathered_stats is not None:
            assert gathered_stats.shape == (6, B) and gathered_stats.dtype == torch.float32 and gathered_stats.is_contiguous()
        lib().dclip_distill_loss_rows(_p(s_img), _p(t_img), _p(s_txt), _p(t_txt), B, E, int(row0), nrow,
                                      ctypes.cast(cfg_arr, ctypes.c_void_p), _p(out), _p(d_i), _p(d_t), _p(gathered_stats),
                                      _p(stats), _p(ws), ws_bytes, _stream())
        if stats_only:
            return stats
    return out, d_i, d_t


def interactive_loss(s_img, t_img, s_txt, t_txt, temperature, weight=1.0):
    _chk(s_img, t_img, s_txt, t_txt)
    for t in (s_img, t_img, s_txt, t_txt):
        if t.dtype != torch.float32 or t.dim() != 2 or t.shape != s_img.shape or not t.is_contiguous():
            raise ValueError(f'interactive_loss: need four contiguous f32 [B, E] tensors of one shape, got {tuple(t.shape)} {t.dtype}')
    B, E = s_img.shape
    ws_bytes = lib().dclip_interactive_loss_workspace(B, E)
    if ws_bytes == 0:
        raise ValueError(f'interactive_loss: need 1 <= B <= 4096, E % 16 == 0, 16 <= E <= 1024, got B={B} E={E}')
    ws = torch.empty(ws_bytes, dtype=torch.uint8, device=s_img.device)
    out = torch.empty(4, dtype=torch.float32, device=s_img.device)
    d_i, d_t = torch.empty_like(s_img), torch.empty_like(s_txt)
    lib().dclip_interactive_loss(_p(s_img), _p(t_img), _p(s_txt), _p(t_txt), B, E, float(temperature), float(weight), _p(out), _p(d_i),
                                 _p(d_t), _p(ws), ws_bytes, _stream())
    return out, d_i, d_t


def relation_kl(s, t, temperature, weight=1.0):
    _chk(s, t)
    for x in (s, t):
        if x.dtype != torch.float32 or x.dim() != 2 or x.shape != s.shape or not x.is_contiguous():
            raise ValueError(f'relation_kl: need two contiguous f32 [B, E] tensors of one shape, got {tuple(x.shape)} {x.dtype}')
    B, E = s.shape
    ws_bytes = lib().dclip_relation_kl_workspace(B, E)
    if ws_bytes == 0:
        raise ValueError(f'relation_kl: need 1 <= B <= 4096, E % 16 == 0, 16 <= E <= 1024, got B={B} E={E}')
    ws = torch.empty(ws_bytes, dtype=torch.uint8, device=s.device)
    out = torch.empty(4, dtype=torch.float32, device=s.device)
    d_s = torch.empty_like(s)
    lib().dclip_relation_kl(_p(s), _p(t), B, E, float(temperature), float(weight), _p(out), _p(d_s), _p(ws), ws_bytes, _stream())
    return out, d_s


def attn_fused_fwd(qkv, B, N, H, hd, causal=False):
    _chk(qkv)
    D = H * hd
    ctx = torch.empty((B * N, D), dtype=torch.bfloat16, device=qkv.device)
    lib().dclip_attn_fused_fwd(_p(qkv), qkv.stride(0), _p(ctx), D, B, H, N, hd, hd ** -0.5, 1 if causal else 0, _stream())
    return ctx


def attn_fused_fwd_rows(qkv, ctx, B, N, H, hd, pick, causal=False):
    _chk(qkv, ctx, pick)
    lib().dclip_attn_fused_fwd_rows(_p(qkv), qkv.stride(0), _p(ctx), ctx.stride(0), B, H, N, hd, hd ** -0.5, 1 if causal else 0, _p(pick),
                                    _stream())
    return ctx


def attn_stream_fwd(qkv, B, N, H, hd):
    _chk(qkv)
    D = H * hd
    ctx = torch.empty((B * N, D), dtype=torch.bfloat16, device=qkv.device)
    lib().dclip_attn_stream_fwd(_p(qkv), qkv.stride(0), _p(ctx), D, B, H, N, hd, hd ** -0.5, _stream())
    return ctx


def im2row_ld(image, patch, ldk=None, cls_rows=1):
    _chk(image)
    assert image.dtype == torch.float32 and image.dim() == 4 and image.is_contiguous() and image.shape[2] == image.shape[3]
    B, C, R, _ = image.shape
    K = C * patch * patch
    ldk = (K + 63) // 64 * 64 if ldk is None else int(ldk)
    g = R // patch
    rows = torch.empty((B * (g * g + cls_rows), ldk), dtype=torch.bfloat16, device=image.device)
    lib().dclip_im2row_ld(_p(image), _p(rows), ldk, B, C, R, patch, cls_rows, _stream())
    return rows


def embed_scatter_add(ids, dx, dtable):
    _chk(ids, dx, dtable)
    rows, D = dx.shape
    lib().dclip_embed_scatter_add(_p(ids), _p(dx), 1 if dx.dtype == torch.float32 else 0, _p(dtable), rows, D, dtable.shape[0],
                                  _stream())
    return dtable


def feature_mse(s, t, coef=1.0):
    _chk(s, t)
    assert s.dtype == torch.float32 and t.dtype == torch.float32 and s.numel() == t.numel() and s.numel() % 4 == 0
    val = torch.zeros(1, dtype=torch.float32, device=s.device)
    ds = torch.zeros_like(s)
    lib().dclip_feature_mse(_p(s), _p(t), s.numel(), float(coef), _p(val), _p(ds), _stream())
    return val[0], ds


def attn_mix_fwd(qkv, B, N, H, hd, wl, ww, scale):
    _chk(qkv, wl, ww)
    Np = (N + 7) // 8 * 8
    r = torch.full((B, H, Np // 4, N, 4), float('nan'), dtype=torch.bfloat16, device=qkv.device)
    stats = torch.empty((B, H, N), dtype=torch.float32, device=qkv.device)
    lib().dclip_attn_mix_fwd(_p(qkv), qkv.stride(0), _p(wl), _p(ww), _p(r), _p(stats), B, H, N, Np, hd, scale, _stream())
    return r, stats


def attn_mix_bwd(qkv, d_ctx, B, N, H, hd, wl, ww, stats, scale, dwl, dww):
    _chk(qkv, d_ctx, wl, ww, stats, dwl, dww)
    Np = (N + 7) // 8 * 8
    ds = torch.full((B, H, Np // 4, N, 4), float('nan'), dtype=torch.bfloat16, device=qkv.device)
    ws = torch.empty(lib().dclip_attn_mix_bwd_workspace_bytes(B, H, N), dtype=torch.uint8, device=qkv.device)
    lib().dclip_attn_mix_bwd(_p(qkv), qkv.stride(0), _p(d_ctx), d_ctx.stride(0), _p(wl), _p(ww), _p(stats), _p(ds), _p(dwl), _p(dww),
                             _p(ws), ws.numel(), B, H, N, Np, hd, scale, _stream())
    return ds


def attn_mix_fwd_rows(qkv, r, stats, wl, ww, scale, pick):
    _chk(qkv, r, stats, wl, ww, pick)
    B, H, N, Np, _ = _score_dims(r)
    lib().dclip_attn_mix_fwd_rows(_p(qkv), qkv.stride(0), _p(wl), _p(ww), _p(r), _p(stats), B, H, N, Np, qkv.shape[1] // (3 * H), scale,
                                  _p(pick), _stream())


def attn_mix_bwd_rows(qkv, d_ctx, ds, wl, ww, stats, scale, dwl, dww, pick, ws=None):
    _chk(qkv, d_ctx, ds, wl, ww, stats, dwl, dww, pick)
    B, H, N, Np, _ = _score_dims(ds)
    if ws is None:
        ws = torch.empty(lib().dclip_attn_mix_bwd_workspace_bytes(B, H, N), dtype=torch.uint8, device=qkv.device)
    lib().dclip_attn_mix_bwd_rows(_p(qkv), qkv.stride(0), _p(d_ctx), d_ctx.stride(0), _p(wl), _p(ww), _p(stats), _p(ds), _p(dwl), _p(dww),
                                  _p(ws), ws.numel(), B, H, N, Np, qkv.shape[1] // (3 * H), scale, _p(pick), _stream())


def cast_transpose_multi(ws, want_b=True, want_t=True):
    import ctypes
    _chk(*ws)
    n = len(ws)
    wb = [torch.empty_like(w, dtype=torch.bfloat16) for w in ws] if want_b else [None] * n
    wt = [torch.empty((w.shape[1], w.shape[0]), dtype=torch.bfloat16, device=w.device) for w in ws] if want_t else [None] * n
    arr = lambda ts: (ctypes.c_void_p * n)(*[None if t is None else t.data_ptr() for t in ts])
    R = (ctypes.c_int64 * n)(*[w.shape[0] for w in ws])
    C = (ctypes.c_int64 * n)(*[w.shape[1] for w in ws])
    lib().dclip_cast_transpose_bf16_multi(arr(ws), arr(wb), arr(wt), R, C, n, _stream())
    return (wb if want_b else None), (wt if want_t else None)


SUMSQ_PARTIALS = 1024
ADAMW_MAX_RANGES = 24


def _range_arrays(items, width):
    import ctypes
    for it in items:
        _chk(*it)
    n = len(items)
    ptrs = [(ctypes.c_void_p * max(n, 1))(*[t[k].data_ptr() for t in items]) for k in range(width)]
    return ptrs, (ctypes.c_int64 * max(n, 1))(*[t[0].numel() for t in items]), n


def sumsq_multi(gs, partials, stream=None):
    _chk(partials)
    (ptrs,), lens, n = _range_arrays([(g,) for g in gs], 1)
    lib().dclip_sumsq_multi(ptrs, lens, n, _p(partials), partials.numel(), _stream() if stream is None else stream)
    return partials


def clip_coef(partials, max_norm, out, extra_sumsq=None, stream=None):
    _chk(partials, extra_sumsq, out)
    lib().dclip_clip_coef(_p(partials), partials.numel(), _p(extra_sumsq), float(max_norm), _p(out), _stream() if stream is None else stream)
    return out


def adamw_multi_scaled(items, lr, betas, eps, weight_decay, step, zero_grad=False, gscale=None, stream=None):
    ptrs, lens, n = _range_arrays(items, 4)
    _chk(gscale)
    lib().dclip_adamw_multi_scaled(*ptrs, lens, n, lr, betas[0], betas[1], eps, weight_decay, step,
                                   1 if zero_grad else 0, _p(gscale), _stream() if stream is None else stream)


AMP_RECORD_FLOATS = 8
AMP_MULT, AMP_SKIP, AMP_BC1, AMP_BC2_SQRT, AMP_NORM, AMP_COEF = range(6)


def amp_prepare(record, skipped, betas, step, found_inf=None, grad_scale=None, partials=None, max_norm=0.0, extra_sumsq=None, stream=None):
    _chk(record, skipped, found_inf, grad_scale, partials, extra_sumsq)
    for t in (found_inf, grad_scale):
        if t is not None and (t.dtype != torch.float32 or t.numel() != 1):
            raise ValueError('amp_prepare: found_inf and grad_scale are 1-element f32 tensors')
    if record.dtype != torch.float32 or record.numel() < AMP_RECORD_FLOATS or skipped.dtype != torch.int64:
        raise ValueError('amp_prepare: record is %d f32, skipped one int64' % AMP_RECORD_FLOATS)
    lib().dclip_amp_prepare(_p(found_inf), _p(grad_scale), _p(partials), 0 if partials is None else partials.numel(), _p(extra_sumsq), float(max_norm),
                            betas[0], betas[1], step, _p(skipped), _p(record), _stream() if stream is None else stream)
    return record


def adamw_multi_amp(items, lr, betas, eps, weight_decay, zero_grad, record, stream=None):
    ptrs, lens, n = _range_arrays(items, 4)
    _chk(record)
    lib().dclip_adamw_multi_amp(*ptrs, lens, n, lr, betas[0], betas[1], eps, weight_decay, 1 if zero_grad else 0,
                                _p(record), _stream() if stream is None else stream)


def adamw_multi_ema(items, lr, betas, eps, weight_decay, step, zero_grad, ema_weight, gscale=None, record=None, stream=None):
    ptrs, lens, n = _range_arrays(items, 5)
    _chk(gscale, record)
    lib().dclip_adamw_multi_ema(*ptrs, lens, n, lr, betas[0], betas[1], eps, weight_decay, step,
                                1 if zero_grad else 0, ema_weight, _p(gscale), _p(record), _stream() if stream is None else stream)


ADAMW_TABLE_TILE = 8192


def adamw_table_image(ranges, total, out=None):
    import ctypes
    n = len(ranges)
    need = lib().dclip_adamw_table_bytes(n)
    if out is None:
        out = torch.zeros(max(need, 8), dtype=torch.uint8)
    if out.is_cuda or out.dtype != torch.uint8 or not out.is_contiguous():
        raise ValueError('adamw_table_image: out is a contiguous CPU uint8 tensor')
    col = lambda k, ct: (ct * max(n, 1))(*[r[k] for r in ranges])
    tiles = ctypes.c_int64(0)
    lib().dclip_adamw_table_fill(col(0, ctypes.c_int64), col(1, ctypes.c_int64), col(2, ctypes.c_float), col(3, ctypes.c_float), n, total,
                                 out.data_ptr(), out.numel(), ctypes.byref(tiles))
    return out, tiles.value


def _table_operands(what, p, g, m, v, e, table, count):
    if table.dtype != torch.uint8 or table.numel() < lib().dclip_adamw_table_bytes(count):
        raise ValueError('%s: table is the uint8 device copy of an image of %d ranges' % (what, count))
    if any(t.numel() != p.numel() or t.dtype != torch.float32 for t in (p, g, m, v) + (() if e is None else (e,))):
        raise ValueError('%s: p, g, m, v (and e) are f32 buffers of one length, the `total` the table was filled for' % what)


def adamw_table(p, g, m, v, e, table, count, tiles, lr, betas, eps, step, zero_grad=False, ema_weight=0.0, gscale=None, record=None, stream=None):
    _chk(p, g, m, v, e, table, gscale, record)
    _table_operands('adamw_table', p, g, m, v, e, table, count)
    lib().dclip_adamw_table(_p(p), _p(g), _p(m), _p(v), _p(e), _p(table), count, tiles, lr, betas[0], betas[1], eps, step, 1 if zero_grad else 0,
                            ema_weight, _p(gscale), _p(record), _stream() if stream is None else stream)


def lamb_buffers(count, tiles, device):
    return (torch.empty(max(lib().dclip_lamb_workspace_bytes(count, tiles), 16), dtype=torch.uint8, device=device),
            torch.zeros(count, 4, dtype=torch.float32, device=device))


def lamb_table(p, g, m, v, e, table, count, tiles, lr, betas, eps, step, workspace, stats, zero_grad=False, ema_weight=0.0, gscale=None, record=None,
               trust_clip=None, always_adapt=False, stream=None):
    _chk(p, g, m, v, e, table, gscale, record, workspace, stats)
    _table_operands('lamb_table', p, g, m, v, e, table, count)
    if workspace.dtype != torch.uint8 or stats.dtype != torch.float32 or stats.numel() < 4 * count:
        raise ValueError('lamb_table: workspace is uint8, stats f32 [%d, 4] (lamb_buffers)' % count)
    lib().dclip_lamb_table(_p(p), _p(g), _p(m), _p(v), _p(e), _p(table), count, tiles, lr, betas[0], betas[1], eps, step, 1 if zero_grad else 0,
                           ema_weight, _p(gscale), _p(record), -1.0 if trust_clip is None else float(trust_clip), 1 if always_adapt else 0,
                           _p(workspace), workspace.numel(), _p(stats), _stream() if stream is None else stream)


def swap_multi(pairs, stream=None):
    for a, b in pairs:
        _chk(a, b)
        if a.numel() != b.numel():
            raise ValueError('swap_multi: the two sides of a pair have %d and %d elements' % (a.numel(), b.numel()))
    ptrs, lens, n = _range_arrays(pairs, 2)
    lib().dclip_swap_multi(*ptrs, lens, n, _stream() if stream is None else stream)


def clipscore(img, cand, refs=None, ref_offsets=None, *, K=1, w=2.5):
    _chk(img, cand, refs, ref_offsets)
    if (refs is None) != (ref_offsets is None):
        raise ValueError('clipscore: refs and ref_offsets come together')
    for name, t in (('img', img), ('cand', cand), ('refs', refs)):
        if t is not None and (t.dtype != torch.float32 or t.dim() != 2 or t.stride(1) != 1):
            raise ValueError(f'clipscore: {name} must be an f32 [rows, E] matrix with unit column stride')
    B, E = img.shape
    K = int(K)
    if K < 1 or cand.shape != (B * K, E) or (refs is not None and refs.shape[1] != E):
        raise ValueError(f'clipscore: img {tuple(img.shape)} and K={K} need cand [{B * K}, {E}] and refs [R, {E}], got {tuple(cand.shape)}'
                         + ('' if refs is None else f' and {tuple(refs.shape)}'))
    R = 0
    if refs is not None:
        if ref_offsets.dtype != torch.int32 or ref_offsets.dim() != 1 or ref_offsets.numel() != B + 1 or not ref_offsets.is_contiguous():
            raise ValueError(f'clipscore: ref_offsets must be a contiguous int32 [{B + 1}] tensor')
        R = refs.shape[0]
        if R == 0:
            refs = img.new_zeros((1, E))
    clip_s = torch.empty(B * K, dtype=torch.float32, device=img.device)
    ref_s = torch.empty_like(clip_s) if refs is not None else None
    refclip_s = torch.empty_like(clip_s) if refs is not None else None
    lib().dclip_clipscore(_p(img), img.stride(0), _p(cand), cand.stride(0), _p(refs), 0 if refs is None else refs.stride(0),
                          _p(ref_offsets), B, K, R, E, float(w), _p(clip_s), _p(ref_s), _p(refclip_s), _stream())
    return clip_s, ref_s, refclip_s
```

### include/dclip.h

```cpp
#ifndef DCLIP_H
#define DCLIP_H
#include <stddef.h>
#include <stdint.h>
#ifdef __cplusplus
extern "C" {
#endif

#define DCLIP_OK 0
#define DCLIP_EINVAL (-1)
#define DCLIP_ELAUNCH (-2)

int dclip_version(void);
int dclip_runtime_check(void);
const char* dclip_arch(void);
const char* dclip_last_error_string(void);

#define DCLIP_ACT_NONE 0
#define DCLIP_ACT_QUICKGELU 1
#define DCLIP_ACT_GELU 2
#define DCLIP_ACT_DGELU 3
#define DCLIP_ACT_MULAUX 4
#define DCLIP_ACT_GELU_SAVE 5
#define DCLIP_ACT_QUICKGELU_SAVE 6
#define DCLIP_OUT_BF16 0
#define DCLIP_OUT_F32 1
#define DCLIP_OUT_F16 2

int dclip_gemm_nt(const void* A, int64_t lda, const void* B, int64_t ldb, void* C, int64_t ldc,
                  int64_t M, int64_t N, int64_t K, float alpha, const float* bias, int act,
                  const void* aux_in, void* aux_out, const void* residual, int64_t ldr, int out_dtype,
                  int64_t row_group, const float* rowadd, float* colsum_acc, void* stream);

size_t dclip_gemm_tn_workspace_bytes(void);
int64_t dclip_gemm_tn_atomic_fallbacks(void);
int dclip_gemm_tn_acc(const void* A, int64_t lda, const void* B, int64_t ldb, float* dW, int64_t ldo,
                      int64_t M, int64_t P, int64_t Q, int splits, void* workspace, size_t ws_bytes, void* stream);

int dclip_colsum_acc(const void* X, int64_t ld, float* db, int64_t M, int64_t N, void* stream);

int dclip_layernorm_fwd(const float* x, int64_t ldx, const int32_t* row_index, const float* gamma, const float* beta,
                        void* y, int64_t ldy, int out_f32, float* mean, float* rstd, int64_t M, int64_t D, float eps,
                        void* stream);
int dclip_layernorm_fwd_f16(const void* x, int64_t ldx, const int32_t* row_index, const float* gamma, const float* beta,
                            void* y, int64_t ldy, int out_dtype, float* mean, float* rstd, int64_t M, int64_t D, float eps,
                            void* stream);
int dclip_layernorm_bwd(const void* dy, int64_t lddy, int dy_f32, const float* x, int64_t ldx, const int32_t* row_index,
                        const float* gamma, const float* mean, const float* rstd, float* dx_acc, int64_t lddx,
                        void* dx_bf16, int64_t lddb, float* dgamma, float* dbeta, float* colsum_acc, int64_t M, int64_t D,
                        void* stream);

int dclip_attn_nt(const void* A, int64_t lda, const void* Bm, int64_t ldb, void* C, int out_f32, int64_t B, int64_t H,
                  int64_t N, int64_t Np, int64_t hd, float alpha, void* stream);
int dclip_attn_nn(const void* A, const void* Bm, int64_t ldb, void* C, int64_t ldc, int64_t B, int64_t H, int64_t N,
                  int64_t Np, int64_t hd, float alpha, int a_blocked, void* stream);
int dclip_attn_tn(const void* A, const void* Bm, int64_t ldb, void* C, int64_t ldc, int64_t B, int64_t H, int64_t N,
                  int64_t Np, int64_t hd, float alpha, int a_blocked, void* stream);
int dclip_attn_fused_fwd(const void* qkv, int64_t ldq, void* ctx, int64_t ldc, int64_t B, int64_t H, int64_t N, int64_t hd,
                         float scale, int causal, void* stream);
int dclip_attn_stream_fwd(const void* qkv, int64_t ldq, void* ctx, int64_t ldc, int64_t B, int64_t H, int64_t N, int64_t hd,
                          float scale, void* stream);
int dclip_attn_softmax_fwd(const float* S, const float* Wl, const float* Ww, void* P, void* R, int64_t B, int64_t H,
                           int64_t N, int64_t Np, int causal, void* stream);
int dclip_attn_softmax_bwd(const void* dR, const void* P, const void* S, int scores_bf16, const float* Wl, const float* Ww,
                           void* dS, float* dWl, float* dWw, int64_t B, int64_t H, int64_t N, int64_t Np, void* stream);
int dclip_attn_mix_supported(int64_t H, int64_t N, int64_t hd);
size_t dclip_attn_mix_bwd_workspace_bytes(int64_t B, int64_t H, int64_t N);
void dclip_attn_mix_debug_stamps(void* fwd, void* bwd_a, void* bwd_b);
int dclip_attn_mix_fwd(const void* qkv, int64_t ld, const float* Wl, const float* Ww, void* R, float* stats, int64_t B, int64_t H,
                       int64_t N, int64_t Np, int64_t hd, float scale, void* stream);
int dclip_attn_mix_bwd(const void* qkv, int64_t ld, const void* dO, int64_t ldo, const float* Wl, const float* Ww,
                       const float* stats, void* dS, float* dWl, float* dWw, void* workspace, size_t ws_bytes, int64_t B, int64_t H,
                       int64_t N, int64_t Np, int64_t hd, float scale, void* stream);
int dclip_attn_nn_rows(const void* A, const void* Bm, int64_t ldb, void* C, int64_t ldc, int64_t B, int64_t H, int64_t N, int64_t Np,
                       int64_t hd, float alpha, int a_blocked, const int32_t* pick, int fill_zero, void* stream);
int dclip_attn_tn_rows(const void* A, const void* Bm, int64_t ldb, void* C, int64_t ldc, int64_t B, int64_t H, int64_t N, int64_t Np,
                       int64_t hd, float alpha, int a_blocked, const int32_t* pick, void* stream);
int dclip_attn_fused_fwd_rows(const void* qkv, int64_t ldq, void* ctx, int64_t ldc, int64_t B, int64_t H, int64_t N, int64_t hd,
                              float scale, int causal, const int32_t* pick, void* stream);
int dclip_attn_mix_fwd_rows(const void* qkv, int64_t ld, const float* Wl, const float* Ww, void* R, float* stats, int64_t B, int64_t H,
                            int64_t N, int64_t Np, int64_t hd, float scale, const int32_t* pick, void* stream);
int dclip_attn_mix_bwd_rows(const void* qkv, int64_t ld, const void* dO, int64_t ldo, const float* Wl, const float* Ww,
                            const float* stats, void* dS, float* dWl, float* dWw, void* workspace, size_t ws_bytes, int64_t B, int64_t H,
                            int64_t N, int64_t Np, int64_t hd, float scale, const int32_t* pick, void* stream);
int dclip_attn_maps_fwd(const void* qkv, int64_t ld, const float* Wl, float* score_map, float* prob_map, int64_t B, int64_t H, int64_t N,
                        int64_t hd, float scale, int causal, void* stream);
size_t dclip_attn_maps_bwd_workspace_bytes(int64_t B, int64_t H, int64_t N);
int dclip_attn_maps_bwd(const void* qkv, int64_t ld, const float* Wl, const float* d_score_map, const float* d_prob_map, void* dS,
                        int ds_blocked, float* dWl, void* workspace, size_t ws_bytes, int64_t B, int64_t H, int64_t N, int64_t Np,
                        int64_t hd, float scale, int causal, void* stream);

int dclip_cast_bf16(const float* src, void* dst, int64_t n, void* stream);
int dclip_cast_f16_f32(const void* src, float* dst, int64_t n, void* stream);
int dclip_axpy_f32(float* dst, const float* src, void* dst_bf16, int64_t n, float* colsum_acc, int64_t D, void* stream);
int dclip_cast_transpose_bf16_multi(const float* const* W, void* const* Wb, void* const* Wt, const int64_t* R, const int64_t* C,
                                    int64_t n, void* stream);
int dclip_im2row(const float* img, void* rows, int64_t B, int64_t C, int64_t res, int64_t patch, int cls_rows, void* stream);
int dclip_im2row_ld(const float* img, void* rows, int64_t ldk, int64_t B, int64_t C, int64_t res, int64_t patch, int cls_rows,
                    void* stream);
int dclip_token_table(const float* pos, const float* cls, const float* bias, float* out, int64_t ntok, int64_t D, void* stream);
int dclip_token_table_bwd(const float* tok_sum, float* dpos, float* dcls, float* dbias, int64_t ntok, int64_t D, int has_cls,
                          void* stream);
int dclip_batch_sum_acc(const float* G, float* out, int64_t B, int64_t N, int64_t D, void* stream);
int dclip_embed_gather(const int64_t* ids, int64_t id_stride, const float* table, const float* pos, void* out, int out_dtype,
                       int64_t rows, int64_t N, int64_t D, void* stream);
int dclip_embed_scatter_add(const int64_t* ids, const void* dx, int dx_f32, float* dtable, int64_t rows, int64_t D,
                            int64_t vocab, void* stream);
int dclip_pick_index(const int64_t* ids, int64_t id_stride, int32_t* idx, int64_t B, int64_t N, void* stream);
int dclip_adamw(float* p, float* g, float* m, float* v, int64_t n, float lr, float beta1, float beta2, float eps,
                float weight_decay, int64_t step, int zero_grad, void* stream);
#define DCLIP_ADAMW_MAX_RANGES 24
int dclip_adamw_multi(float* const* p, float* const* g, float* const* m, float* const* v, const int64_t* n, int32_t count, float lr,
                      float beta1, float beta2, float eps, float weight_decay, int64_t step, int zero_grad, void* stream);
int dclip_adamw_multi_scaled(float* const* p, float* const* g, float* const* m, float* const* v, const int64_t* n, int32_t count,
                             float lr, float beta1, float beta2, float eps, float weight_decay, int64_t step, int zero_grad,
                             const float* gscale, void* stream);
#define DCLIP_SUMSQ_PARTIALS 1024
int dclip_sumsq_multi(const float* const* g, const int64_t* n, int32_t count, float* partials, int64_t n_partials, void* stream);
int dclip_clip_coef(const float* partials, int64_t n_partials, const float* extra_sumsq, float max_norm, float* out, void* stream);
#define DCLIP_AMP_RECORD_FLOATS 8
#define DCLIP_AMP_MULT 0
#define DCLIP_AMP_SKIP 1
#define DCLIP_AMP_BC1 2
#define DCLIP_AMP_BC2_SQRT 3
#define DCLIP_AMP_NORM 4
#define DCLIP_AMP_COEF 5
int dclip_amp_prepare(const float* found_inf, const float* grad_scale, const float* partials, int64_t n_partials, const float* extra_sumsq,
                      float max_norm, float beta1, float beta2, int64_t step, int64_t* skipped, float* record, void* stream);
int dclip_adamw_multi_amp(float* const* p, float* const* g, float* const* m, float* const* v, const int64_t* n, int32_t count, float lr,
                          float beta1, float beta2, float eps, float weight_decay, int zero_grad, const float* record, void* stream);
int dclip_adamw_multi_ema(float* const* p, float* const* g, float* const* m, float* const* v, float* const* e, const int64_t* n, int32_t count,
                          float lr, float beta1, float beta2, float eps, float weight_decay, int64_t step, int zero_grad, float ema_weight,
                          const float* gscale, const float* record, void* stream);
int dclip_swap_multi(float* const* a, float* const* b, const int64_t* n, int32_t count, void* stream);
#define DCLIP_ADAMW_TABLE_TILE 8192
typedef struct dclip_adamw_range {
    int64_t tile0;
    int64_t begin, length;
    float lr_scale, weight_decay;
} dclip_adamw_range;
size_t dclip_adamw_table_bytes(int32_t count);
int dclip_adamw_table_fill(const int64_t* begin, const int64_t* length, const float* lr_scale, const float* weight_decay, int32_t count,
                           int64_t total, void* image, size_t image_bytes, int64_t* tiles);
int dclip_adamw_table(float* p, float* g, float* m, float* v, float* e, const void* table, int32_t count, int64_t tiles, float lr, float beta1,
                      float beta2, float eps, int64_t step, int zero_grad, float ema_weight, const float* gscale, const float* record,
                      void* stream);
size_t dclip_lamb_workspace_bytes(int32_t count, int64_t tiles);
int dclip_lamb_table(float* p, float* g, float* m, float* v, float* e, const void* table, int32_t count, int64_t tiles, float lr, float beta1,
                     float beta2, float eps, int64_t step, int zero_grad, float ema_weight, const float* gscale, const float* record,
                     float trust_clip, int always_adapt, void* workspace, size_t ws_bytes, float* stats, void* stream);

size_t dclip_distill_loss_workspace(int64_t B, int64_t E);
int dclip_distill_loss(const float* s_img, const float* t_img, const float* s_txt, const float* t_txt, int64_t B, int64_t E,
                       const float* cfg, float* out_scalars, float* d_s_img, float* d_s_txt, void* workspace,
                       size_t ws_bytes, void* stream);
typedef struct dclip_aug_op {
    int32_t op;
    int32_t c[6];
    float f;
} dclip_aug_op;
size_t dclip_augment_workspace(int64_t B, int64_t H, int64_t W);
int dclip_augment_normalize(const uint8_t* images, int64_t B, int64_t H, int64_t W, const dclip_aug_op* ops, int num_ops,
                            const float* mean3, const float* std3, float* out, uint8_t* aug_out, void* workspace,
                            size_t ws_bytes, void* stream);
typedef struct dclip_resize_desc {
    int64_t src_offset;
    int64_t table_offset;
    int64_t temp_offset;
    int32_t height, width;
    int32_t row0, nrows;
    int32_t ksize_h, ksize_v;
} dclip_resize_desc;
int dclip_resize_center_crop(const uint8_t* packed, const dclip_resize_desc* desc, const int32_t* tables, int64_t B, int64_t S,
                             uint8_t* out, void* workspace, size_t ws_bytes, void* stream);
size_t dclip_retrieval_metrics_workspace(int64_t n, int64_t E);
int dclip_retrieval_metrics(const float* img, const float* txt, int64_t n, int64_t E, const int32_t* ks, int nk,
                            float* out, int32_t* rank_out, void* workspace, size_t ws_bytes, void* stream);
size_t dclip_retrieval_recall_workspace(int64_t n_img, int64_t n_txt, int64_t E);
int dclip_retrieval_recall(const float* img, const float* txt, const int32_t* txt_offsets, int64_t n_img, int64_t n_txt, int64_t E,
                           const int32_t* ks, int nk, float* out, int32_t* rank_i2t, int32_t* rank_t2i, void* workspace, size_t ws_bytes,
                           void* stream);
size_t dclip_topk_search_workspace(int64_t nq, int64_t ng, int64_t E, int k);
int dclip_topk_search(const float* queries, const float* gallery, int64_t nq, int64_t ng, int64_t E, int k, int32_t* idx, float* score,
                      void* workspace, size_t ws_bytes, void* stream);
int dclip_group_mean_rows(const float* rows, const int32_t* offsets, int64_t n_groups, int64_t n_rows, int64_t E, float* out,
                          void* stream);
int dclip_clipscore(const float* img, int64_t ld_img, const float* cand, int64_t ld_cand, const float* refs, int64_t ld_ref,
                    const int32_t* ref_offsets, int64_t B, int64_t K, int64_t R, int64_t E, float w, float* clip_s, float* ref_s,
                    float* refclip_s, void* stream);
size_t dclip_kendall_tau_workspace(int64_t n, int64_t C);
int dclip_kendall_tau(const float* scores, int64_t ld, int64_t C, const float* human, int64_t n, double* out_tau, int64_t* out_counts,
                      void* workspace, size_t ws_bytes, void* stream);
size_t dclip_rank_correlation_workspace(int64_t n, int64_t C);
int dclip_rank_correlation(const float* scores, int64_t ld, int64_t C, const float* human, int64_t n, double* out_corr, int64_t* out_sums,
                           int32_t* out_ranks, void* workspace, size_t ws_bytes, void* stream);
int dclip_distill_loss_rows(const float* s_img, const float* t_img, const float* s_txt, const float* t_txt, int64_t B, int64_t E,
                            int64_t row0, int64_t rows, const float* cfg, float* out_scalars, float* d_s_img, float* d_s_txt,
                            const float* gathered_stats, float* stats_out, void* workspace, size_t ws_bytes, void* stream);
int dclip_feature_mse(const float* s, const float* t, int64_t n, float coef, float* loss_acc, float* ds_acc, void* stream);
size_t dclip_interactive_loss_workspace(int64_t B, int64_t E);
int dclip_interactive_loss(const float* s_img, const float* t_img, const float* s_txt, const float* t_txt, int64_t B, int64_t E,
                           float tau, float weight, float* out, float* d_s_img, float* d_s_txt, void* workspace, size_t ws_bytes,
                           void* stream);
size_t dclip_relation_kl_workspace(int64_t B, int64_t E);
int dclip_relation_kl(const float* s, const float* t, int64_t B, int64_t E, float tau, float weight, float* out, float* d_s,
                      void* workspace, size_t ws_bytes, void* stream);

typedef struct dclip_encoder_cfg {
    int32_t kind;
    int32_t modality;
    int32_t tokens;
    int32_t width;
    int32_t heads;
    int32_t layers;
    int32_t repeats;
    int32_t mlp_dim;
    int32_t out_dim;
    int32_t patch, resolution, in_chans;
    int32_t vocab, embed_rank;
    int32_t head_mix;
    int32_t causal;
} dclip_encoder_cfg;

typedef struct dclip_encoder dclip_encoder;

dclip_encoder* dclip_encoder_create(const dclip_encoder_cfg* cfg);
void dclip_encoder_destroy(dclip_encoder* enc);
int64_t dclip_encoder_num_params(const dclip_encoder* enc);
size_t dclip_encoder_wcache_bytes(const dclip_encoder* enc);
size_t dclip_encoder_workspace_bytes(const dclip_encoder* enc, int64_t B, int training);
int dclip_encoder_prepare(const dclip_encoder* enc, const void* const* params, void* wcache, void* stream);
typedef struct dclip_attn_maps {
    int32_t n;
    const int32_t* exec;
    float* const* score;
    float* const* prob;
    const float* const* d_score;
    const float* const* d_prob;
    void* scratch;
    size_t scratch_bytes;
} dclip_attn_maps;
typedef struct dclip_encoder_run {
    uint32_t flags;
    uint32_t reserved;
    uint64_t score_maps;
    uint64_t prob_maps;
} dclip_encoder_run;
int dclip_encoder_forward(const dclip_encoder* enc, const void* input, const void* patches, int64_t B, const void* const* params,
                          const void* wcache, void* workspace, size_t ws_bytes, dclip_encoder_run* run, int training,
                          float* last_representation, float* const* rep_out, float* emb_out, int64_t tokens_eff,
                          const dclip_attn_maps* maps, void* stream);
size_t dclip_encoder_last_layer_output_scratch_bytes(const dclip_encoder* enc, int64_t B, int training);
int dclip_encoder_last_layer_output(const dclip_encoder* enc, int64_t B, const void* const* params, const void* wcache,
                                    void* workspace, size_t ws_bytes, const dclip_encoder_run* run, int training, void* scratch,
                                    float* out, void* stream);
typedef void (*dclip_bucket_cb)(void* user, int32_t bucket);
int dclip_encoder_backward(const dclip_encoder* enc, const void* input, const void* patches, int64_t B, const void* const* params,
                           void* const* grads, const void* wcache, void* workspace, size_t ws_bytes, dclip_encoder_run* run,
                           const float* d_last_representation, const float* const* d_rep, const float* d_emb,
                           const dclip_attn_maps* maps, dclip_bucket_cb on_bucket, void* cb_user, void* stream);
int32_t dclip_encoder_num_grad_buckets(const dclip_encoder* enc);
int dclip_encoder_grad_bucket(const dclip_encoder* enc, int32_t bucket, int32_t* first_param, int32_t* end_param);

int dclip_trace_begin(int64_t max_records);
int64_t dclip_trace_end(int32_t* kind, float* ms, double* flops, double* bytes, int64_t cap);
int64_t dclip_trace_dims(int32_t* dims, int64_t cap);
int dclip_trace_gemm_stamps(void* buf);
int dclip_trace_attn_stamps(void* buf);
int64_t dclip_trace_gemm_clock(void* buf, int64_t cap);

#ifdef __cplusplus
}
#endif
#endif
```

Measured before the change: 18550 pairs/s.

## Add single-row fused mix-attention kernels for pruned last layer

```diff
diff --git a/distillclip_amd/csrc/attention_mix.hip b/distillclip_amd/csrc/attention_mix.hip
--- a/distillclip_amd/csrc/attention_mix.hip
+++ b/distillclip_amd/csrc/attention_mix.hip
@@ -233,6 +233,13 @@
 
 }
 
+extern "C" int dclip_attn_mix_wgrad_reduce(const void* partial, int nwg, int64_t H, float* dWl, float* dWw, void* stream) {
+    DCLIP_REQUIRE(partial && dWl && dWw && nwg >= 1 && nwg <= BWD_MAX_WG && H >= 1, "dclip_attn_mix_wgrad_reduce: bad argument");
+    hipLaunchKernelGGL(attn_mix_wgrad_reduce_kernel, dim3((unsigned)(2 * H * H)), dim3(256), 0, (hipStream_t)stream, (const float*)partial, nwg,
+                       (int)H, (int)((H + 15) / 16) * 16, dWl, dWw);
+    return dclip_check_launch("dclip_attn_mix_wgrad_reduce");
+}
+
 extern "C" int dclip_attn_mix_fwd(const void* qkv, int64_t ld, const float* Wl, const float* Ww, void* R, float* stats, int64_t B,
                                   int64_t H, int64_t N, int64_t Np, int64_t hd, float scale, void* stream) {
     return launch_mix_fwd("dclip_attn_mix_fwd", qkv, ld, Wl, Ww, R, stats, B, H, N, Np, hd, scale, nullptr, stream);
diff --git a/distillclip_amd/csrc/attention_row.hip b/distillclip_amd/csrc/attention_row.hip
--- /dev/null
+++ b/distillclip_amd/csrc/attention_row.hip
@@ -0,0 +1,400 @@
+#include <math.h>
+#include "common.h"
+
+#define DEVFN __device__ __forceinline__
+
+namespace {
+
+constexpr float LOG2E = 1.4426950408889634f;
+constexpr float LN2 = 0.6931471805599453f;
+constexpr int ROW_MAX_WG = 256;
+constexpr int FWD_NT = 512, BWD_NT = 1024;
+constexpr int MAX_GROUPS = 10;
+
+template <int H_, int HD_>
+struct Cfg {
+    static constexpr int H = H_, HD = HD_;
+    static constexpr int D = H * HD;
+    static constexpr int CH = D / 8;
+    static constexpr int CPH = HD / 8;
+    static constexpr int HP = 16 * ((H + 15) / 16);
+};
+template <class C, int NT> constexpr int groups() { return NT / C::CH < MAX_GROUPS ? NT / C::CH : MAX_GROUPS; }
+constexpr int group_slots(int G) { return (G + 1) / 2; }
+
+DEVFN int row_ld(int Np) { return Np + 1; }
+
+struct RowArgs {
+    const bf16_t* qkv; long ld;
+    const float* Wl; const float* Ww;
+    bf16_t* R;
+    float* stats;
+    const int32_t* pick;
+    bf16_t* ctx; long ldc;
+    const bf16_t* dO; long ldo;
+    bf16_t* dqkv; long ldg;
+    float* partial;
+    int B, N, Np;
+    float scale;
+};
+
+DEVFN int picked_row(const int32_t* pick, int b, int N) {
+    const int n = pick[b] - b * N;
+    return __builtin_amdgcn_readfirstlane(min(max(n, 0), N - 1));
+}
+
+template <class C, int NT, bool ROUND_BF16>
+DEVFN void dot_rows(const bf16_t* mat, long ld, int N, const bf16_t* vec, float* out, int ldo, int tid) {
+    const int total = N * C::CH;
+    constexpr int U = NT >= 1024 ? 4 : 8;
+    for (int base = 0; base < total; base += U * NT) {
+        bf16x8 k[U];
+#pragma unroll
+        for (int u = 0; u < U; ++u) {
+            const int idx = base + u * NT + tid;
+            const int j = idx / C::CH, c = idx - j * C::CH;
+            k[u] = *(const bf16x8*)(mat + (long)(idx < total ? j : N - 1) * ld + 8 * c);
+        }
+#pragma unroll
+        for (int u = 0; u < U; ++u) {
+            const int idx = base + u * NT + tid;
+            const int j = idx / C::CH, c = idx - j * C::CH;
+            const bf16x8 q = *(const bf16x8*)(vec + 8 * c);
+            float s = 0.f;
+#pragma unroll
+            for (int e = 0; e < 8; ++e) s = fmaf((float)k[u][e], (float)q[e], s);
+#pragma unroll
+            for (int o = 1; o < C::CPH; o <<= 1) s += __shfl_xor(s, o);
+            if (idx < total && (c % C::CPH) == 0) out[(c / C::CPH) * ldo + j] = ROUND_BF16 ? (float)(bf16_t)s : s;
+        }
+    }
+}
+
+template <class C, int NT>
+DEVFN void weighted_rows(const bf16_t* mat, long ld, int N, const float* coef, int ldco, float* part, int tid) {
+    constexpr int G = groups<C, NT>(), SL = group_slots(G);
+    const int grp = tid / C::CH, c = tid - grp * C::CH;
+    float acc[8] = {0.f, 0.f, 0.f, 0.f, 0.f, 0.f, 0.f, 0.f};
+    if (grp < G) {
+        const float* co = coef + (c / C::CPH) * ldco;
+        constexpr int U = NT >= 1024 ? 4 : 8;
+        for (int j0 = grp; j0 < N; j0 += U * G) {
+            bf16x8 v[U];
+#pragma unroll
+            for (int u = 0; u < U; ++u) v[u] = *(const bf16x8*)(mat + (long)min(j0 + u * G, N - 1) * ld + 8 * c);
+#pragma unroll
+            for (int u = 0; u < U; ++u) {
+                const float r = j0 + u * G < N ? co[j0 + u * G] : 0.f;
+#pragma unroll
+                for (int e = 0; e < 8; ++e) acc[e] = fmaf(r, (float)v[u][e], acc[e]);
+            }
+        }
+    }
+    if (grp < SL) {
+#pragma unroll
+        for (int e = 0; e < 8; ++e) part[grp * C::D + 8 * c + e] = acc[e];
+    }
+    __syncthreads();
+    if (grp >= SL && grp < G) {
+#pragma unroll
+        for (int e = 0; e < 8; ++e) part[(grp - SL) * C::D + 8 * c + e] += acc[e];
+    }
+    __syncthreads();
+    for (int d = tid; d < C::D; d += NT) {
+        float s = part[d];
+#pragma unroll
+        for (int g = 1; g < SL; ++g) s += part[g * C::D + d];
+        part[d] = s;
+    }
+    __syncthreads();
+}
+
+template <class C, int NT>
+struct Lds {
+    float *w0, *w1, *w2, *t0, *t1, *t2, *t3, *part, *vh;
+    bf16_t *v0, *v1;
+    DEVFN Lds(char* smem, int Np, bool bwd) {
+        const int ld = row_ld(Np);
+        float* f = (float*)smem;
+        w0 = f; f += C::H * C::H; w1 = f; f += C::H * C::H;
+        w2 = nullptr;
+        if (bwd) { w2 = f; f += C::H * C::H; }
+        t0 = f; f += C::H * ld; t1 = f; f += C::H * ld;
+        t2 = t3 = nullptr;
+        if (bwd) { t2 = f; f += C::H * ld; t3 = f; f += C::H * ld; }
+        vh = f; f += C::H;
+        f = (float*)(((uintptr_t)f + 15) & ~(uintptr_t)15);
+        part = f; f += group_slots(groups<C, NT>()) * C::D;
+        v0 = (bf16_t*)f; v1 = v0 + C::D;
+    }
+};
+size_t lds_bytes(int64_t H, int64_t hd, int threads, int64_t Np, bool bwd) {
+    const size_t D = (size_t)(H * hd), ld = (size_t)Np + 1, nw = bwd ? 3 : 2, nt = bwd ? 4 : 2;
+    const size_t G = threads / (D / 8) < MAX_GROUPS ? threads / (D / 8) : MAX_GROUPS;
+    return (nw * H * H + nt * H * ld + H) * 4 + 16 + (size_t)group_slots((int)G) * D * 4 + 2 * D * 2;
+}
+
+template <class C>
+DEVFN float mix1(const float* w, const float* S, int ld, int g, int j, float init) {
+    float a = init;
+#pragma unroll
+    for (int h = 0; h < C::H; ++h) a = fmaf(w[g * C::H + h], (float)(_Float16)S[h * ld + j], a);
+    return a;
+}
+
+template <int H, int HD>
+__global__ __launch_bounds__(FWD_NT) void attn_mix_fwd_row_kernel(RowArgs p) {
+    using C = Cfg<H, HD>;
+    constexpr int NT = FWD_NT, D = C::D;
+    extern __shared__ __attribute__((aligned(16))) char smem[];
+    const Lds<C, NT> L(smem, p.Np, false);
+    const int tid = threadIdx.x, lane = tid & 63, wave = tid >> 6;
+    const int b = blockIdx.x, N = p.N, Np = p.Np, ld = row_ld(Np);
+    const int n = picked_row(p.pick, b, N);
+    const bf16_t* base = p.qkv + (long)b * N * p.ld;
+    float* wl = L.w0; float* ww = L.w1; float* S = L.t0; float* T = L.t1;
+    const float sc = p.scale * LOG2E;
+    for (int i = tid; i < H * H; i += NT) {
+        wl[i] = (float)(_Float16)(p.Wl[i] * sc);
+        ww[i] = (float)(_Float16)p.Ww[i];
+    }
+    for (int c = tid; c < C::CH; c += NT) *(bf16x8*)(L.v0 + 8 * c) = *(const bf16x8*)(base + (long)n * p.ld + 8 * c);
+    __syncthreads();
+    dot_rows<C, NT, false>(base + D, p.ld, N, L.v0, S, ld, tid);
+    __syncthreads();
+    for (int g = wave; g < H; g += NT / 64) {
+        float a[2], m = -INFINITY;
+#pragma unroll
+        for (int u = 0; u < 2; ++u) {
+            const int j = lane + 64 * u;
+            a[u] = j < N ? mix1<C>(wl, S, ld, g, j, 0.f) : -INFINITY;
+            m = fmaxf(m, a[u]);
+        }
+        m = wave_max(m);
+        float l = 0.f;
+#pragma unroll
+        for (int u = 0; u < 2; ++u) l += lane + 64 * u < N ? __builtin_amdgcn_exp2f(a[u] - m) : 0.f;
+        l = wave_sum(l);
+        const float lse2 = m + __builtin_amdgcn_logf(l);
+        if (lane == 0) p.stats[((long)b * H + g) * N + n] = lse2 * LN2;
+#pragma unroll
+        for (int u = 0; u < 2; ++u) {
+            const int j = lane + 64 * u;
+            if (j < N) T[g * ld + j] = (float)(_Float16)__builtin_amdgcn_exp2f(a[u] - lse2);
+        }
+    }
+    __syncthreads();
+    float* Rr = S;
+    bf16_t* Rg = p.R + (long)b * H * N * Np;
+    for (int idx = tid; idx < H * Np; idx += NT) {
+        const int g = idx / Np, j = idx - g * Np;
+        float r = 0.f;
+        if (j < N) {
+#pragma unroll
+            for (int h = 0; h < H; ++h) r = fmaf(ww[g * H + h], T[h * ld + j], r);
+        }
+        const bf16_t rb = (bf16_t)r;
+        Rr[g * ld + j] = (float)rb;
+        Rg[(long)g * N * Np + ((long)(j >> 2) * N + n) * 4 + (j & 3)] = rb;
+    }
+    __syncthreads();
+    weighted_rows<C, NT>(base + 2 * D, p.ld, N, Rr, ld, L.part, tid);
+    for (int c = tid; c < C::CH; c += NT) {
+        bf16x8 o;
+#pragma unroll
+        for (int e = 0; e < 8; ++e) o[e] = f2bf(L.part[8 * c + e] * 1.f);
+        *(bf16x8*)(p.ctx + (long)b * p.ldc + 8 * c) = o;
+    }
+}
+
+template <int H, int HD>
+__global__ __launch_bounds__(BWD_NT) void attn_mix_bwd_row_kernel(RowArgs p) {
+    using C = Cfg<H, HD>;
+    constexpr int NT = BWD_NT, D = C::D, HP = C::HP, CH = C::CH, CPH = C::CPH;
+    constexpr int WPT = (H * H + NT - 1) / NT;
+    extern __shared__ __attribute__((aligned(16))) char smem[];
+    const Lds<C, NT> L(smem, p.Np, true);
+    const int tid = threadIdx.x, lane = tid & 63, wave = tid >> 6;
+    const int N = p.N, Np = p.Np, ld = row_ld(Np);
+    float* wl = L.w0;
+    float* wwt = L.w1;
+    float* wlt = L.w2;
+    float* S = L.t0;
+    float* P = L.t1;
+    float* dR = L.t2;
+    float* dA = L.t3;
+    float* nlse = L.vh;
+    bf16_t* qrow = L.v0; bf16_t* dorow = L.v1;
+    const float sc = p.scale * LOG2E;
+    for (int i = tid; i < H * H; i += NT) {
+        wl[i] = (float)(_Float16)(p.Wl[i] * sc);
+        wwt[i] = (float)(bf16_t)p.Ww[i];
+        wlt[i] = (float)(bf16_t)p.Wl[i];
+    }
+    float gl[WPT], gw[WPT];
+#pragma unroll
+    for (int k = 0; k < WPT; ++k) gl[k] = gw[k] = 0.f;
+
+    for (int b = blockIdx.x; b < p.B; b += gridDim.x) {
+        const int n = picked_row(p.pick, b, N);
+        const bf16_t* base = p.qkv + (long)b * N * p.ld;
+        bf16_t* gbase = p.dqkv + (long)b * N * p.ldg;
+        __syncthreads();
+        for (int c = tid; c < 2 * CH; c += NT) {
+            if (c < CH) *(bf16x8*)(qrow + 8 * c) = *(const bf16x8*)(base + (long)n * p.ld + 8 * c);
+            else *(bf16x8*)(dorow + 8 * (c - CH)) = *(const bf16x8*)(p.dO + (long)b * p.ldo + 8 * (c - CH));
+        }
+        for (int g = tid; g < H; g += NT) nlse[g] = -p.stats[((long)b * H + g) * N + n] * LOG2E;
+        __syncthreads();
+        dot_rows<C, NT, false>(base + D, p.ld, N, qrow, S, ld, tid);
+        dot_rows<C, NT, true>(base + 2 * D, p.ld, N, dorow, dR, ld, tid);
+        __syncthreads();
+        for (int idx = tid; idx < H * N; idx += NT) {
+            const int h = idx / N, j = idx - h * N;
+            P[h * ld + j] = __builtin_amdgcn_exp2f(mix1<C>(wl, S, ld, h, j, nlse[h]));
+            float dp = 0.f;
+#pragma unroll
+            for (int g = 0; g < H; ++g) dp = fmaf(wwt[g * H + h], dR[g * ld + j], dp);
+            dA[h * ld + j] = dp;
+        }
+        __syncthreads();
+        for (int h = wave; h < H; h += NT / 64) {
+            float pr[2], dp[2], dl = 0.f;
+#pragma unroll
+            for (int u = 0; u < 2; ++u) {
+                const int j = lane + 64 * u;
+                pr[u] = j < N ? P[h * ld + j] : 0.f;
+                dp[u] = j < N ? dA[h * ld + j] : 0.f;
+                dl = fmaf(pr[u], dp[u], dl);
+            }
+            dl = wave_sum(dl);
+#pragma unroll
+            for (int u = 0; u < 2; ++u) {
+                const int j = lane + 64 * u;
+                if (j < N) dA[h * ld + j] = (float)(bf16_t)(pr[u] * (dp[u] - dl));
+            }
+        }
+        __syncthreads();
+#pragma unroll
+        for (int k = 0; k < WPT; ++k) {
+            const int e = tid + k * NT;
+            if (e < H * H) {
+                const int g = e / H, h = e - g * H;
+                float aw = 0.f, al = 0.f;
+                for (int j = 0; j < N; ++j) {
+                    aw = fmaf(dR[g * ld + j], (float)(bf16_t)P[h * ld + j], aw);
+                    al = fmaf(dA[g * ld + j], (float)(bf16_t)(S[h * ld + j] * p.scale), al);
+                }
+                gw[k] += aw;
+                gl[k] += al;
+            }
+        }
+        __syncthreads();
+        const bf16_t* Rg = p.R + (long)b * H * N * Np;
+        for (int idx = tid; idx < H * N; idx += NT) {
+            const int h = idx / N, j = idx - h * N;
+            float ds = 0.f;
+#pragma unroll
+            for (int g = 0; g < H; ++g) ds = fmaf(wlt[g * H + h], dA[g * ld + j], ds);
+            S[h * ld + j] = (float)(bf16_t)ds;
+            P[h * ld + j] = (float)Rg[(long)h * N * Np + ((long)(j >> 2) * N + n) * 4 + (j & 3)];
+        }
+        __syncthreads();
+        const int total = N * CH;
+        for (int idx = tid; idx < total; idx += NT) {
+            const int j = idx / CH, c = idx - j * CH, h = c / CPH;
+            const bf16x8 q = *(const bf16x8*)(qrow + 8 * c), d = *(const bf16x8*)(dorow + 8 * c);
+            const float r = P[h * ld + j], s = S[h * ld + j];
+            bf16x8 ov, ok;
+#pragma unroll
+            for (int e = 0; e < 8; ++e) {
+                ov[e] = f2bf(r * (float)d[e] * 1.f);
+                ok[e] = f2bf(s * (float)q[e] * p.scale);
+            }
+            bf16_t* row = gbase + (long)j * p.ldg + 8 * c;
+            *(bf16x8*)(row + 2 * D) = ov;
+            *(bf16x8*)(row + D) = ok;
+            if (j != n) *(bf16x8*)row = bf16x8{};
+        }
+        weighted_rows<C, NT>(base + D, p.ld, N, S, ld, L.part, tid);
+        for (int c = tid; c < CH; c += NT) {
+            bf16x8 o;
+#pragma unroll
+            for (int e = 0; e < 8; ++e) o[e] = f2bf(L.part[8 * c + e] * p.scale);
+            *(bf16x8*)(gbase + (long)n * p.ldg + 8 * c) = o;
+        }
+    }
+    float* out = p.partial + (long)blockIdx.x * 2 * HP * HP;
+#pragma unroll
+    for (int k = 0; k < WPT; ++k) {
+        const int e = tid + k * NT;
+        if (e < H * H) {
+            const int g = e / H, h = e - g * H;
+            out[g * HP + h] = gl[k];
+            out[HP * HP + g * HP + h] = gw[k];
+        }
+    }
+}
+
+}
+
+#define ROW_DISPATCH(Hv, HDv, ...)                                                     \
+    switch ((Hv) * 100 + (HDv)) {                                                      \
+        case 232: { constexpr int HH = 2, HD_ = 32; typedef Cfg<HH, HD_> CC; __VA_ARGS__; break; }              \
+        case 264: { constexpr int HH = 2, HD_ = 64; typedef Cfg<HH, HD_> CC; __VA_ARGS__; break; }              \
+        case 432: { constexpr int HH = 4, HD_ = 32; typedef Cfg<HH, HD_> CC; __VA_ARGS__; break; }              \
+        case 464: { constexpr int HH = 4, HD_ = 64; typedef Cfg<HH, HD_> CC; __VA_ARGS__; break; }              \
+        case 832: { constexpr int HH = 8, HD_ = 32; typedef Cfg<HH, HD_> CC; __VA_ARGS__; break; }              \
+        case 864: { constexpr int HH = 8, HD_ = 64; typedef Cfg<HH, HD_> CC; __VA_ARGS__; break; }              \
+        case 1232: { constexpr int HH = 12, HD_ = 32; typedef Cfg<HH, HD_> CC; __VA_ARGS__; break; }            \
+        case 1264: { constexpr int HH = 12, HD_ = 64; typedef Cfg<HH, HD_> CC; __VA_ARGS__; break; }            \
+        case 2432: { constexpr int HH = 24, HD_ = 32; typedef Cfg<HH, HD_> CC; __VA_ARGS__; break; }            \
+        default: dclip_set_error("attn_mix_row: no instantiation for H=%d hd=%d", (int)(Hv), (int)(HDv)); return DCLIP_EINVAL; \
+    }
+
+extern "C" int dclip_attn_mix_row_supported(int64_t H, int64_t N, int64_t hd) {
+    if (!dclip_attn_mix_supported(H, N, hd)) return 0;
+    return lds_bytes(H, hd, BWD_NT, (N + 7) & ~(int64_t)7, true) <= 65536;
+}
+
+extern "C" int dclip_attn_mix_fwd_row(const void* qkv, int64_t ld, const float* Wl, const float* Ww, void* R, float* stats, void* ctx,
+                                      int64_t ldc, int64_t B, int64_t H, int64_t N, int64_t Np, int64_t hd, float scale, const int32_t* pick,
+                                      void* stream) {
+    const char* who = "dclip_attn_mix_fwd_row";
+    DCLIP_REQUIRE(qkv && Wl && Ww && R && stats && ctx && pick && B > 0, "%s: null / empty argument", who);
+    DCLIP_REQUIRE(dclip_attn_mix_row_supported(H, N, hd), "%s: unsupported shape H=%ld N=%ld hd=%ld", who, (long)H, (long)N, (long)hd);
+    DCLIP_REQUIRE(Np == ((N + 7) & ~(int64_t)7) && ld % 8 == 0 && ldc % 8 == 0 && ld >= 3 * H * hd && ldc >= H * hd && dclip_aligned16(qkv) &&
+                      dclip_aligned16(ctx) && dclip_aligned16(R),
+                  "%s: misaligned buffers (Np = round_up(N, 8), 16-byte aligned qkv and ctx rows and R)", who);
+    RowArgs p{(const bf16_t*)qkv, (long)ld, Wl, Ww, (bf16_t*)R, stats, pick, (bf16_t*)ctx, (long)ldc, nullptr, 0, nullptr, 0, nullptr,
+              (int)B, (int)N, (int)Np, scale};
+    TraceScope tr(DCLIP_TRACE_ATTN, 4.0 * B * H * N * hd + 4.0 * B * H * H * N, 4.0 * B * N * H * hd, stream, (int)(B * H), (int)N, (int)hd, 9);
+    ROW_DISPATCH(H, hd, hipLaunchKernelGGL((attn_mix_fwd_row_kernel<HH, HD_>), dim3((unsigned)B), dim3(FWD_NT), lds_bytes(H, hd, FWD_NT, Np, false),
+                                           (hipStream_t)stream, p));
+    return dclip_check_launch(who);
+}
+
+extern "C" int dclip_attn_mix_bwd_row(const void* qkv, int64_t ld, const void* dO, int64_t ldo, const float* Wl, const float* Ww, const void* R,
+                                      const float* stats, void* dqkv, int64_t ldg, float* dWl, float* dWw, void* workspace, size_t ws_bytes,
+                                      int64_t B, int64_t H, int64_t N, int64_t Np, int64_t hd, float scale, const int32_t* pick, void* stream) {
+    const char* who = "dclip_attn_mix_bwd_row";
+    DCLIP_REQUIRE(qkv && dO && Wl && Ww && R && stats && dqkv && dWl && dWw && workspace && pick && B > 0, "%s: null / empty argument", who);
+    DCLIP_REQUIRE(dclip_attn_mix_row_supported(H, N, hd), "%s: unsupported shape H=%ld N=%ld hd=%ld", who, (long)H, (long)N, (long)hd);
+    DCLIP_REQUIRE(Np == ((N + 7) & ~(int64_t)7) && ld % 8 == 0 && ldo % 8 == 0 && ldg % 8 == 0 && ld >= 3 * H * hd && ldo >= H * hd &&
+                      ldg >= 3 * H * hd && dclip_aligned16(qkv) && dclip_aligned16(dO) && dclip_aligned16(dqkv) && dclip_aligned16(R) &&
+                      dclip_aligned16(workspace),
+                  "%s: misaligned buffers", who);
+    DCLIP_REQUIRE(ws_bytes >= dclip_attn_mix_bwd_workspace_bytes(B, H, N), "%s: workspace too small (%zu < %zu)", who, ws_bytes,
+                  dclip_attn_mix_bwd_workspace_bytes(B, H, N));
+    const char* g0 = (const char*)dqkv; const char* g1 = g0 + ((size_t)(B * N - 1) * ldg + 3 * H * hd) * 2;
+    const char* o0 = (const char*)dO; const char* o1 = o0 + ((size_t)(B - 1) * ldo + H * hd) * 2;
+    DCLIP_REQUIRE(o1 <= g0 || o0 >= g1, "%s: dO overlaps dqkv", who);
+    const int blocks = (int)(B < ROW_MAX_WG ? B : ROW_MAX_WG);
+    RowArgs p{(const bf16_t*)qkv, (long)ld, Wl, Ww, (bf16_t*)R, (float*)stats, pick, nullptr, 0, (const bf16_t*)dO, (long)ldo, (bf16_t*)dqkv,
+              (long)ldg, (float*)workspace, (int)B, (int)N, (int)Np, scale};
+    TraceScope tr(DCLIP_TRACE_ATTN, 10.0 * B * H * N * hd + 10.0 * B * H * H * N, 12.0 * B * N * H * hd, stream, (int)(B * H), (int)N, (int)hd, 10);
+    ROW_DISPATCH(H, hd, hipLaunchKernelGGL((attn_mix_bwd_row_kernel<HH, HD_>), dim3((unsigned)blocks), dim3(BWD_NT), lds_bytes(H, hd, BWD_NT, Np, true),
+                                           (hipStream_t)stream, p));
+    if (int rc = dclip_check_launch(who)) return rc;
+    return dclip_attn_mix_wgrad_reduce(workspace, blocks, H, dWl, dWw, stream);
+}
diff --git a/distillclip_amd/csrc/common.h b/distillclip_amd/csrc/common.h
--- a/distillclip_amd/csrc/common.h
+++ b/distillclip_amd/csrc/common.h
@@ -27,6 +27,8 @@
 
 extern "C" int dclip_rows_pick(const void* src, void* dst, const int32_t* idx, int64_t B, int64_t row_bytes, void* stream);
 extern "C" int dclip_rows_expand(const void* src, void* dst, const int32_t* idx, int64_t B, int64_t N, int64_t row_bytes, void* stream);
+
+extern "C" int dclip_attn_mix_wgrad_reduce(const void* partial, int nwg, int64_t H, float* dWl, float* dWw, void* stream);
 
 extern "C" int dclip_cast_bf16_pad(const float* src, void* dst, int64_t R, int64_t C, int64_t ldd, void* stream);
 
diff --git a/distillclip_amd/csrc/encoder.cpp b/distillclip_amd/csrc/encoder.cpp
--- a/distillclip_amd/csrc/encoder.cpp
+++ b/distillclip_amd/csrc/encoder.cpp
@@ -299,9 +299,10 @@
 }
 
 int attn_forward(AttnPath path, const Plan& p, const ExecSave& s, const float* wl, const float* ww, int64_t B, int64_t N, const int32_t* pick,
-                 void* st) {
+                 bf16_t* ctx_row, void* st) {
     const int64_t D = p.D, H = p.H, hd = p.hd, Np = (N + 7) & ~(int64_t)7;
     const float scale = 1.f / sqrtf((float)hd);
+    if (ctx_row) return dclip_attn_mix_fwd_row(s.qkv, 3 * D, wl, ww, s.Rm, s.stats, ctx_row, D, B, H, N, Np, hd, scale, pick, st);
     if (path == AttnPath::Fused) {
         if (N <= 128 && pick) return dclip_attn_fused_fwd_rows(s.qkv, 3 * D, s.ctx, D, B, H, N, hd, scale, p.c.causal, pick, st);
         if (N <= 128) return dclip_attn_fused_fwd(s.qkv, 3 * D, s.ctx, D, B, H, N, hd, scale, p.c.causal, st);
@@ -353,7 +354,7 @@
 
 }
 
-enum : uint32_t { RUN_SEEDS_CLEAR = 1u, RUN_PRUNED = 2u, RUN_PRUNED_ATTN = 4u };
+enum : uint32_t { RUN_SEEDS_CLEAR = 1u, RUN_PRUNED = 2u, RUN_PRUNED_ATTN = 4u, RUN_ROW_ATTN = 8u };
 
 struct dclip_encoder { Plan p; };
 
@@ -397,11 +398,11 @@
 }
 
 int exec_attn(const Plan& p, AttnPath path, const ExecSave& s, const bf16_t* W, int l, const EP& e, bool h16, const void* xin, int64_t B,
-              int64_t N, const int32_t* pick, void* st) {
+              int64_t N, const int32_t* pick, bf16_t* ctx_row, void* st) {
     const int64_t D = p.D, M = B * N;
     CK(ln_stream(h16, xin, D, nullptr, e.n1w, e.n1b, s.h1, D, DCLIP_OUT_BF16, s.mean1, s.rstd1, M, D, st));
     CK(gemm(s.h1, D, W + p.bw[l].qkv, D, s.qkv, 3 * D, M, 3 * D, D, e.bq, 0, nullptr, nullptr, nullptr, 0, DCLIP_OUT_BF16, 0, nullptr, st));
-    return attn_forward(path, p, s, e.wl, e.ww, B, N, pick, st);
+    return attn_forward(path, p, s, e.wl, e.ww, B, N, pick, ctx_row, st);
 }
 
 int exec_mlp(const Plan& p, const bf16_t* W, int l, const EP& e, bool h16, const RowSet& rs, void* st) {
@@ -434,9 +435,9 @@
     static const int v = [] { const char* e = getenv("DCLIP_PRUNE_LAST"); return e ? atoi(e) : 1; }();
     return v != 0;
 }
-inline bool prune_attn_enabled() {
-    static const int v = [] { const char* e = getenv("DCLIP_PRUNE_ATTN"); return e ? atoi(e) : 1; }();
-    return v != 0;
+inline int prune_attn_mode() {
+    static const int v = [] { const char* e = getenv("DCLIP_PRUNE_ATTN"); return e ? atoi(e) : 2; }();
+    return v;
 }
 
 template <class T> struct ExecMaps { std::vector<T*> score, prob; uint64_t score_bits = 0, prob_bits = 0; };
@@ -551,7 +552,8 @@
 
     CK(dclip_pick_index(p.image ? nullptr : (const int64_t*)input, p.N, w.pick, B, N, st));
     const bool prune = prune_last_enabled() && !(rep_out && rep_out[nex - 1]) && !xm.score[nex - 1] && !xm.prob[nex - 1];
-    const bool prune_attn = prune && prune_attn_enabled() && N <= 128;
+    const bool prune_attn = prune && prune_attn_mode() != 0 && N <= 128;
+    const bool row_attn = prune_attn && prune_attn_mode() != 1 && w.path == AttnPath::Mix && dclip_attn_mix_row_supported(p.H, N, p.hd) != 0;
     for (int ei = 0; ei < nex; ++ei) {
         const int l = ei / p.R, r = ei % p.R;
         const ExecSave& s = w.ex[ei];
@@ -559,10 +561,11 @@
         const bool compact = prune && ei == nex - 1;
         ExecSave sa = s;
         if (compact) sa.ctx = w.ctx_full;
-        CK(exec_attn(p, w.path, sa, W, l, ep, w.h16, w.X[ei], B, N, compact && prune_attn ? w.pick : nullptr, st));
+        CK(exec_attn(p, w.path, sa, W, l, ep, w.h16, w.X[ei], B, N, compact && prune_attn ? w.pick : nullptr,
+                     compact && row_attn ? w.compact.ctx : nullptr, st));
         if (xm.score[ei] || xm.prob[ei]) CK(dclip_attn_maps_fwd(s.qkv, 3 * D, ep.wl, xm.score[ei], xm.prob[ei], B, p.H, N, p.hd, 1.f / sqrtf((float)p.hd), p.c.causal, st));
         if (compact) {
-            CK(dclip_rows_pick(w.ctx_full, w.compact.ctx, w.pick, B, D * 2, st));
+            if (!row_attn) CK(dclip_rows_pick(w.ctx_full, w.compact.ctx, w.pick, B, D * 2, st));
             CK(dclip_rows_pick(w.X[ei], w.compact.xin, w.pick, B, D * (w.h16 ? 2 : 4), st));
         }
         CK(exec_mlp(p, W, l, ep, w.h16, compact ? w.compact : full_rows(w, ei, M), st));
@@ -572,7 +575,7 @@
     CK(ln_stream(w.h16, prune ? w.compact.xout : w.X[nex], D, prune ? nullptr : w.pick, PF(params, p.head.norm_w), PF(params, p.head.norm_b), w.hf, D,
                  DCLIP_OUT_BF16, w.meanf, w.rstdf, B, D, st));
     CK(gemm(w.hf, D, W + p.w_head, D, last_representation, E, B, E, D, PF(params, p.head.head_b), 0, nullptr, nullptr, nullptr, 0, DCLIP_OUT_F32, 0, nullptr, st));
-    *run = dclip_encoder_run{(prune ? RUN_PRUNED : 0u) | (prune_attn ? RUN_PRUNED_ATTN : 0u), 0, 0, 0};
+    *run = dclip_encoder_run{(prune ? RUN_PRUNED : 0u) | (prune_attn ? RUN_PRUNED_ATTN : 0u) | (row_attn ? RUN_ROW_ATTN : 0u), 0, 0, 0};
     if (training) {
         CK(clear_backward_seeds(p, w, M, B, prune, st));
         run->flags |= RUN_SEEDS_CLEAR;
@@ -610,7 +613,7 @@
         const int ei = nex - 1, l = ei / p.R;
         llo_scratch(p, w.path, w.h16, B, scratch, w.X[ei], t, rs);
         const EP ep = exec_params(p, params, l, ei % p.R);
-        CK(exec_attn(p, w.path, t, W, l, ep, w.h16, w.X[ei], B, p.N, nullptr, st));
+        CK(exec_attn(p, w.path, t, W, l, ep, w.h16, w.X[ei], B, p.N, nullptr, nullptr, st));
         CK(exec_mlp(p, W, l, ep, w.h16, rs, st));
         xlast = rs.xout;
     }
@@ -694,8 +697,14 @@
                                GR(bx.n2w), GR(bx.n2b), GR(bx.prb), Mx, D, st));
         if (r == 0 && GR(bx.prw)) CK(dclip_gemm_tn_acc(w.gb_pr, D, s0.ctx, D, GR(bx.prw), D, MRw, D, D, wsplits(MRw, D, D), w.tn_ws, w.tn_ws_bytes, st));
         bf16_t* dctx = w.dh;
+        const bool row_attn = compact && (run->flags & RUN_ROW_ATTN) != 0;
         if (!compact) {
             CK(gemm(gb_pr, D, W + bw.proj_t, D, dctx, D, M, D, D, nullptr, 0, nullptr, nullptr, nullptr, 0, DCLIP_OUT_BF16, 0, nullptr, st));
+        } else if (row_attn) {
+            CK(gemm(gb_pr, D, W + bw.proj_t, D, dctx, D, B, D, D, nullptr, 0, nullptr, nullptr, nullptr, 0, DCLIP_OUT_BF16, 0, nullptr, st));
+            CK(dclip_rows_expand(w.Gc, w.G, w.pick, B, N, D * 4, st));
+            CK(dclip_attn_mix_bwd_row(s.qkv, 3 * D, dctx, D, wl, ww, s.Rm, s.stats, dqkv, 3 * D, gl ? gl : w.wg_dummy, gw ? gw : w.wg_dummy + p.H * p.H,
+                                      w.mix_ws, w.mix_ws_bytes, B, p.H, N, p.Np, p.hd, 1.f / sqrtf((float)p.hd), w.pick, st));
         } else {
             bf16_t* dctx_c = dqkv;
             CK(gemm(gb_pr, D, W + bw.proj_t, D, dctx_c, D, B, D, D, nullptr, 0, nullptr, nullptr, nullptr, 0, DCLIP_OUT_BF16, 0, nullptr, st));
@@ -703,8 +712,8 @@
             CK(dclip_rows_expand(w.Gc, w.G, w.pick, B, N, D * 4, st));
         }
         const MapGrad mg{gm.score[ei], gm.prob[ei], maps ? maps->scratch : nullptr, maps ? maps->scratch_bytes : 0};
-        CK(attn_backward(w.path, p, s, w, wl, ww, gl, gw, dctx, dqkv, B, mg.d_score || mg.d_prob ? &mg : nullptr,
-                         compact && (run->flags & RUN_PRUNED_ATTN) ? w.pick : nullptr, st));
+        if (!row_attn) CK(attn_backward(w.path, p, s, w, wl, ww, gl, gw, dctx, dqkv, B, mg.d_score || mg.d_prob ? &mg : nullptr,
+                                        compact && (run->flags & RUN_PRUNED_ATTN) ? w.pick : nullptr, st));
         if (r == 0 && GR(bx.qkvw)) CK(dclip_gemm_tn_acc(w.dqkv, 3 * D, s0.h1, D, GR(bx.qkvw), D, MR, 3 * D, D, wsplits(MR, 3 * D, D), w.tn_ws, w.tn_ws_bytes, st));
         if (r == 0 && params[bx.qkvb] && GR(bx.qkvb)) CK(dclip_colsum_acc(w.dqkv, 3 * D, GR(bx.qkvb), MR, 3 * D, st));
         CK(gemm(dqkv, 3 * D, W + bw.qkv_t, 3 * D, w.dh, D, M, D, 3 * D, nullptr, 0, nullptr, nullptr, nullptr, 0, DCLIP_OUT_BF16, 0, nullptr, st));
diff --git a/distillclip_amd/ops.py b/distillclip_amd/ops.py
--- a/distillclip_amd/ops.py
+++ b/distillclip_amd/ops.py
@@ -313,6 +313,23 @@
                                   _p(ws), ws.numel(), B, H, N, Np, qkv.shape[1] // (3 * H), scale, _p(pick), _stream())
 
 
+def attn_mix_fwd_row(qkv, r, stats, ctx, wl, ww, scale, pick):
+    _chk(qkv, r, stats, ctx, wl, ww, pick)
+    B, H, N, Np, _ = _score_dims(r)
+    lib().dclip_attn_mix_fwd_row(_p(qkv), qkv.stride(0), _p(wl), _p(ww), _p(r), _p(stats), _p(ctx), ctx.stride(0), B, H, N, Np,
+                                 qkv.shape[1] // (3 * H), scale, _p(pick), _stream())
+
+
+def attn_mix_bwd_row(qkv, d_ctx, r, stats, dqkv, wl, ww, scale, dwl, dww, pick, ws=None):
+    _chk(qkv, d_ctx, r, stats, dqkv, wl, ww, dwl, dww, pick)
+    B, H, N, Np, _ = _score_dims(r)
+    if ws is None:
+        ws = torch.empty(lib().dclip_attn_mix_bwd_workspace_bytes(B, H, N), dtype=torch.uint8, device=qkv.device)
+    lib().dclip_attn_mix_bwd_row(_p(qkv), qkv.stride(0), _p(d_ctx), d_ctx.stride(0), _p(wl), _p(ww), _p(r), _p(stats), _p(dqkv),
+                                 dqkv.stride(0), _p(dwl), _p(dww), _p(ws), ws.numel(), B, H, N, Np, qkv.shape[1] // (3 * H), scale, _p(pick),
+                                 _stream())
+
+
 def cast_transpose_multi(ws, want_b=True, want_t=True):
     import ctypes
     _chk(*ws)
diff --git a/include/dclip.h b/include/dclip.h
--- a/include/dclip.h
+++ b/include/dclip.h
@@ -82,6 +82,12 @@
 int dclip_attn_mix_bwd_rows(const void* qkv, int64_t ld, const void* dO, int64_t ldo, const float* Wl, const float* Ww,
                             const float* stats, void* dS, float* dWl, float* dWw, void* workspace, size_t ws_bytes, int64_t B, int64_t H,
                             int64_t N, int64_t Np, int64_t hd, float scale, const int32_t* pick, void* stream);
+int dclip_attn_mix_row_supported(int64_t H, int64_t N, int64_t hd);
+int dclip_attn_mix_fwd_row(const void* qkv, int64_t ld, const float* Wl, const float* Ww, void* R, float* stats, void* ctx, int64_t ldc,
+                           int64_t B, int64_t H, int64_t N, int64_t Np, int64_t hd, float scale, const int32_t* pick, void* stream);
+int dclip_attn_mix_bwd_row(const void* qkv, int64_t ld, const void* dO, int64_t ldo, const float* Wl, const float* Ww, const void* R,
+                           const float* stats, void* dqkv, int64_t ldg, float* dWl, float* dWw, void* workspace, size_t ws_bytes, int64_t B,
+                           int64_t H, int64_t N, int64_t Np, int64_t hd, float scale, const int32_t* pick, void* stream);
 int dclip_attn_maps_fwd(const void* qkv, int64_t ld, const float* Wl, float* score_map, float* prob_map, int64_t B, int64_t H, int64_t N,
                         int64_t hd, float scale, int causal, void* stream);
 size_t dclip_attn_maps_bwd_workspace_bytes(int64_t B, int64_t H, int64_t N);
```

New measurement: 18720 pairs/s (median of 6 runs). No clear change (+0.9%).
